# google/lyra

Measured on AMD Instinct MI355X. Metric: 20ms 16kHz frames/sec encode+decode (whole node) at batch 4096; xRT/stream, higher is better.
Workload: dtype f32+i8 (fp32 and int8 layers exactly as the reference graphs)

## Files before the change

lyra_amd/csrc/dec_kernels.hip:

```cpp
#include "dec_stages.h"

#ifdef LYRA_TIMING
extern "C" int lyra_hip_debug_exit_at_d0(int i) {
  return (int)hipMemcpyToSymbol(HIP_SYMBOL(g_lyra_exit_at), &i, sizeof(int));
}
extern "C" int lyra_hip_debug_timing_d0(long long* out) {
  return (int)hipMemcpyFromSymbol(out, HIP_SYMBOL(g_lyra_tdbg), sizeof(long long) * 128);
}
extern "C" int lyra_hip_debug_wgtrace_d0(long long* out) {
  return (int)hipMemcpyFromSymbol(out, HIP_SYMBOL(g_lyra_wgtrace), sizeof(long long) * 2048 * 4);
}
#endif

namespace lyra {

size_t dec_s0_lds_bytes() { return dec_s0_lds(); }
int dec_s0_streams_per_wg() { return SD0; }

__global__ __launch_bounds__(NTD0, I8_WAVES) void dec_s0_kernel(const DecS0P* __restrict__ Pp, const float* __restrict__ feats,
                                                       const int32_t* __restrict__ ids, int B,
                                                       uint8_t* __restrict__ state, float* __restrict__ out0,
                                                       const uint8_t* __restrict__ packets, int num_stages,
                                                       const float* __restrict__ cb, int code_bytes, int tile0) {
  LYRA_STRESS(4);
  if (((int)blockIdx.x + tile0) * SD0 >= B) return;
  dec_s0_body<0>(Pp, feats, ids, B, state, out0, packets, num_stages, cb, code_bytes, (int)blockIdx.x + tile0);
}
__global__ __launch_bounds__(NTD0, I8_WAVES) void dec_s0_dr_kernel(const DecS0P* __restrict__ Pp, const float* __restrict__ feats,
                                                          const int32_t* __restrict__ ids, int B,
                                                          uint8_t* __restrict__ state, float* __restrict__ out0,
                                                          const uint8_t* __restrict__ packets, int num_stages,
                                                          const float* __restrict__ cb, int code_bytes, int tile0) {
  LYRA_STRESS(4);
  if (((int)blockIdx.x + tile0) * SD0 >= B) return;
  dec_s0_body<1>(Pp, feats, ids, B, state, out0, packets, num_stages, cb, code_bytes, (int)blockIdx.x + tile0);
}
__global__ __launch_bounds__(NTD0, I8_WAVES) void dec_s0_bm_kernel(const DecS0P* __restrict__ Pp, const float* __restrict__ feats,
                                                          const int32_t* __restrict__ ids, int B,
                                                          uint8_t* __restrict__ state, float* __restrict__ out0,
                                                          const uint8_t* __restrict__ packets, int num_stages,
                                                          const float* __restrict__ cb, int code_bytes, int tile0) {
  LYRA_STRESS(4);
  if (((int)blockIdx.x + tile0) * SD0 >= B) return;
  dec_s0_body<3>(Pp, feats, ids, B, state, out0, packets, num_stages, cb, code_bytes, (int)blockIdx.x + tile0);
}
__global__ __launch_bounds__(NTD0, I8_WAVES) void dec_s0_xn_kernel(const DecS0P* __restrict__ Pp, const float* __restrict__ feats,
                                                          const int32_t* __restrict__ ids, int B,
                                                          uint8_t* __restrict__ state, float* __restrict__ out0,
                                                          const uint8_t* __restrict__ packets, int num_stages,
                                                          const float* __restrict__ cb, int code_bytes, int tile0) {
  LYRA_STRESS(4);
  if (((int)blockIdx.x + tile0) * SD0 >= B) return;
  dec_s0_body<2>(Pp, feats, ids, B, state, out0, packets, num_stages, cb, code_bytes, (int)blockIdx.x + tile0);
}

size_t dec_s1_lds_bytes() { return dec_s1_lds(); }
int dec_s1_streams_per_wg() { return SD1; }
int dec_s1_threads() { return NTD1; }

__global__ __launch_bounds__(NTD1, NTD1 == 512 ? 4 : 3) void dec_s1_kernel(const DecS1P* __restrict__ Pp, const float* __restrict__ in0,
                                                                          const int32_t* __restrict__ ids, int B,
                                                                          uint8_t* __restrict__ state, float* __restrict__ out1,
                                                                          int code_bytes, int tile0) {
  LYRA_STRESS(5);
  if (((int)blockIdx.x + tile0) * SD1 >= B) return;
  dec_s1_body(*Pp, in0, ids, B, state, out1, code_bytes, (int)blockIdx.x + tile0);
}

namespace {
constexpr int SD2 = S0_STREAMS;
}

size_t dec_s2_lds_bytes() { return dec_s2_lds(SD2); }
int dec_s2_streams_per_wg() { return SD2; }
int dec_s2_threads() { return 64 * SD2; }

__global__ __launch_bounds__(64 * SD2, C64_WAVES) void dec_s2_kernel(const DecS2P* __restrict__ Pp, const float* __restrict__ in1,
                                                            const int32_t* __restrict__ ids, int B,
                                                            uint8_t* __restrict__ state, int16_t* __restrict__ pcm,
                                                            int code_bytes, int tile0) {
  LYRA_STRESS(6);
  if (((int)blockIdx.x + tile0) * SD2 >= B) return;
  dec_s2_body<SD2>(*Pp, in1, ids, B, state, pcm, code_bytes, (int)blockIdx.x + tile0);
}


}
```

lyra_amd/csrc/dec_stages.h:

```cpp
#ifndef LYRA_AMD_CSRC_DEC_STAGES_H_
#define LYRA_AMD_CSRC_DEC_STAGES_H_
#include "resblock_q.h"

namespace lyra {

namespace {
constexpr int SD0 = 8;
constexpr int FS = 72;
constexpr int CS2 = 264;
constexpr int QS = 288;
constexpr int QS5 = 544;
constexpr int NTD0 = 512;
constexpr int MTD0 = (2 * SD0) / 16;
constexpr int FB_FLOATS = 3 * 16 * FS;
constexpr int XF_FLOATS = 2 * SD0 * CS2;
constexpr int H8_BYTES = 16 * QS5;
constexpr int QB_BYTES = 2 * SD0 * QS;
constexpr int QA_BYTES = 2 * 16 * QS;
constexpr int NLR = 6, NADD = 2;
static_assert(SD0 == 8, "tile size the index math below supports");
}

__host__ __device__ constexpr size_t dec_s0_lds() {
  return (size_t)(FB_FLOATS + XF_FLOATS) * 4 + H8_BYTES + 3 * QB_BYTES + QA_BYTES + 2 * SD0 * 4 + NLR * 256 +
         NADD * 2048;
}

template <int MODE>
__device__ __forceinline__ void dec_s0_body(const DecS0P* __restrict__ Pp, const float* __restrict__ feats,
                                            const int32_t* __restrict__ ids, int B, uint8_t* __restrict__ state,
                                            float* __restrict__ out0, const uint8_t* __restrict__ packets, int num_stages,
                                            const float* __restrict__ cb, int code_bytes, int tile = (int)blockIdx.x) {
  const DecS0P& P = *Pp;
  extern __shared__ __attribute__((aligned(16))) float smem[];
  float* FB = smem;
  float* XF = FB + FB_FLOATS;
  int8_t* H8 = reinterpret_cast<int8_t*>(XF + XF_FLOATS);
  int8_t* QX = H8 + H8_BYTES;
  int8_t* QA = QX + QB_BYTES;
  int8_t* QD = QA + QA_BYTES;
  int8_t* QP = QD + QB_BYTES;
  int* sids = reinterpret_cast<int*>(QP + QB_BYTES);
  int* sphase = sids + SD0;
  int32_t* LA = sphase + SD0;
  int8_t* LQ = reinterpret_cast<int8_t*>(LA + NADD * 512);
  const int tid = threadIdx.x, lane = tid & 63, wave = tid >> 6;
  const int m = lane & 15, q = lane >> 4;
  const int b0 = tile * SD0;
  LYRA_TSTAMP(80);
  LYRA_WSTAMP(120);
  LYRA_WG_BEGIN();
  if (tid < SD0) {
    int id = ids[min(b0 + tid, B - 1)];
    sids[tid] = id;
    sphase[tid] = *reinterpret_cast<const int*>(state + (size_t)max(id, 0) * st::D0_BYTES + st::PHASE);
  }
  int pkv = 0;
  const int swave = __builtin_amdgcn_readfirstlane(tid >> 6);
  if (!feats) {
    const int nbytes = (num_stages + 1) >> 1;
    const uint8_t* pk = packets + (size_t)min(b0 + swave, B - 1) * nbytes;
    if (lane < nbytes) pkv = (int)pk[lane];
  }
  load_luts<NTD0>(LQ, P.lr_lut, NLR, LA, P.add_lut, NADD);
  const auto warm = l2_warm<NTD0, 1>(P.warm);
  const auto warm_code = code_warm<NTD0>(code_bytes);
  const auto warm_cb = l2_warm<NTD0, 1>(feats ? WarmRange{nullptr, 0} : WarmRange{reinterpret_cast<const uint8_t*>(cb), 46 * 16 * 64 * 4});
  LYRA_SYNC_KEEP();
  TileCtx cx{state, sids, sphase, B - b0, st::D0_BYTES};
  const uint32_t touch0 = state_touch<SD0, NTD0>(cx, st::D_UP0, 4 * 2 * 64 * 4 + 2 * 256);
  const uint32_t touch1 = state_touch<SD0, NTD0>(cx, st::D_UP1, 2 * 2 * 64 * 4);

  {
    const int c = tid & 63, s = tid >> 6;
    const int b = min(b0 + s, B - 1);
    float f;
    if (feats) {
      f = *goff<const float>(feats + (size_t)b0 * 64, (uint32_t)(((b - b0) * 64 + c) * 4));
    } else {
      f = 0.f;
      const __amdgpu_buffer_rsrc_t cbr = __builtin_amdgcn_make_buffer_rsrc(const_cast<float*>(cb), 0, 46 * 16 * 64 * 4, 0x00020000);
#pragma unroll
      for (int k = 0; k < 46; ++k) {
        const int byte = __builtin_amdgcn_readlane(pkv, k >> 1);
        const int used = (k - num_stages) >> 31;
        const int i = (byte >> ((k & 1) ? 0 : 4)) & 15 & used;
        const float mask = __builtin_bit_cast(float, used & 0x3f800000);
        const float v = __builtin_bit_cast(float, __builtin_amdgcn_raw_buffer_load_b32(cbr, c * 4, (k * 16 + i) * 256, 0));
        f = k == 0 ? v * mask : __builtin_fmaf(v, mask, f);
      }
    }
    FB[(2 * 16 + s) * FS + at16(c)] = f;
  }
  for (int idx = tid; idx < 2 * SD0 * 16; idx += NTD0) {
    int p4 = idx & 15, s = (idx >> 4) & (SD0 - 1), j = (idx >> 4) / SD0;
    int slot = (sphase[s] + j) & 1;
    *reinterpret_cast<f32x4*>(&FB[(j * 16 + s) * FS + p4 * 4]) =
        *cx.at<const f32x4>(cx.soff(s) + (uint32_t)(st::D_HEAD + (slot * 64 + p4 * 4) * 4));
  }
  __syncthreads();
  for (int idx = tid; idx < SD0 * 16; idx += NTD0) {
    int p4 = idx & 15, s = idx >> 4;
    int slot = sphase[s] & 1;
    if (cx.valid(s))
      *cx.at<f32x4>(cx.soff(s) + (uint32_t)(st::D_HEAD + (slot * 64 + p4 * 4) * 4)) =
          *reinterpret_cast<const f32x4*>(&FB[(2 * 16 + s) * FS + p4 * 4]);
  }
  LYRA_TSTAMP(81);
  {
    f32x4 acc[1][4];
    const int g = wave >> 1;
    auto aoff = [&](int i, int c) { return (c * 16 + m) * FS + g * 16 + q * 4; };
    gemm_f32_bias<1, 4, 3, 3>(FB, aoff, P.head.w + (wave * 4) * 3 * 64, P.head.b, wave * 4 * 16, acc);
    fold_rows8<2>(acc[0]);
#pragma unroll
    for (int j = 0; j < 2; ++j) {
      int n = (wave * 4 + j + 2 * (lane >> 5)) * 16 + (lane & 15);
#pragma unroll
      for (int e = 0; e < 4; ++e)
        H8[((q & 1) * 4 + e) * QS5 + n] = (int8_t)quantize_code<MODE>(lrelu(acc[0][j][e]), P.q0);
    }
  }
  __syncthreads();
  LYRA_TSTAMP(82);
  {
    i32x4 acc[1][8];
    const int g = wave >> 1;
    const TconvQ U = P.up0[g];
    auto aoff = [&](int i, int c) { return m * QS5 + g * 128 + c * 64 + q * 16; };
    const int ct = (wave & 1) * 2 + (lane >> 5);
    const int co = ct * 16 + (lane & 15);
    const int bias = as_global(U.bias)[co];
    const float sub = as_global(P.up0_sub[g])[co];
    const int pc = at16(g * 64 + co);
    int zfv[4];
#pragma unroll
    for (int tap = 0; tap < 4; ++tap) zfv[tap] = as_global(U.zfold)[tap * 64 + co];
    float told[2][4];
#pragma unroll
    for (int e = 0; e < 4; ++e) {
      const uint32_t stp = cx.soff((q & 1) * 4 + e) + (uint32_t)(st::D_UP0 + g * 512 + co * 4);
      told[0][e] = *cx.at<const float>(stp);
      told[1][e] = *cx.at<const float>(stp + 256);
    }
    gemm_i8<1, 8, 2>(H8, aoff, U.w + ((wave & 1) * 8) * 2 * 64, acc);
    fold_rows8<4>(acc[0]);
#pragma unroll
    for (int tap = 0; tap < 4; ++tap) {
      const int zf = zfv[tap];
#pragma unroll
      for (int e = 0; e < 4; ++e) {
        const int s = (q & 1) * 4 + e;
        const uint32_t stp = cx.soff(s) + (uint32_t)(st::D_UP0 + g * 512 + co * 4);
        float y = conv_dequant<conv_flavour<MODE, false>()>(acc[0][tap][e] + zf + bias, U.M, U.sh, U.zout, P.up0_dq[g].s);
        if (tap < 2) {
          y = y + told[tap < 2 ? tap : 0][e];
          XF[(tap * SD0 + s) * CS2 + pc] = y;
        } else {
          y = y + 0.f;
          if (cx.valid(s)) *cx.at<float>(stp + (uint32_t)((tap - 2) * 256)) = y - sub;
        }
      }
    }
  }
  __syncthreads();
  LYRA_TSTAMP(83);
  const RbqPre pre1 = resblock_q_prefetch<SD0>(cx, 3, st::D_R0_1, P.dwq[1], P.pwq[1], P.cvq[1]);
  {
    const DwQ dq = P.dwq[0];
    const int w4 = tid & 63, s = tid >> 6;
    const uint32_t hp = cx.soff(s) + (uint32_t)(st::D_R0_0 + w4 * 4);
    const int h0 = *cx.at<const int>(hp), h1 = *cx.at<const int>(hp + 256);
    int ww[3];
#pragma unroll
    for (int j = 0; j < 3; ++j) ww[j] = *reinterpret_cast<const int LYRA_GLOBAL*>(&as_global(dq.w)[j * 256 + w4 * 4]);
    const i32x4 db = *reinterpret_cast<const i32x4 LYRA_GLOBAL*>(&as_global(dq.b)[w4 * 4]);
    const i32x4 dM = *reinterpret_cast<const i32x4 LYRA_GLOBAL*>(&as_global(dq.M)[w4 * 4]);
    const i32x4 dsh = *reinterpret_cast<const i32x4 LYRA_GLOBAL*>(&as_global(dq.sh)[w4 * 4]);
    int a[2];
#pragma unroll
    for (int t = 0; t < 2; ++t) {
      int c8[4];
#pragma unroll
      for (int e = 0; e < 4; ++e)
        c8[e] = quantize_code<MODE>(lrelu(XF[(t * SD0 + s) * CS2 + at16(w4 * 4 + e)]), P.q1);
      a[t] = pack8(c8[0], c8[1], c8[2], c8[3]);
    }
    const int x[2][3] = {{h0, h1, a[0]}, {h1, a[0], a[1]}};
#pragma unroll
    for (int t = 0; t < 2; ++t) {
      int o[4];
#pragma unroll
      for (int e = 0; e < 4; ++e) {
        int acc = db[e];
#pragma unroll
        for (int j = 0; j < 3; ++j) acc += sx8(x[t][j], e) * sx8(ww[j], e);
        o[e] = conv_code<conv_flavour<MODE, false>()>(acc, dM[e], dsh[e], dq.zout);
      }
      *reinterpret_cast<int*>(&QD[(t * SD0 + s) * QS + w4 * 4]) = pack8(o[0], o[1], o[2], o[3]);
      if (cx.valid(s)) *cx.at<int>(hp + (uint32_t)(t * 256)) = a[t];
    }
    __syncthreads();
    LYRA_TSTAMP(84);
    static_assert(MTD0 == 1, "one 16-row M tile: rows (t, s)");
    const int row = lane & 15, ch0 = wave * 32 + q * 4;
    {
      i32x4 acc[2] = {chan_quad(P.pwq[0].b, wave * 2), chan_quad(P.pwq[0].b, wave * 2 + 1)};
      const i32x4 M[2] = {chan_quad(P.pwq[0].M, wave * 2), chan_quad(P.pwq[0].M, wave * 2 + 1)};
      const i32x4 sh[2] = {chan_quad(P.pwq[0].sh, wave * 2), chan_quad(P.pwq[0].sh, wave * 2 + 1)};
      auto aoff = [&](int c) { return m * QS + c * 64 + q * 16; };
      gemm_i8_t<2, 4>(QD, aoff, P.pwq[0].w + (wave * 2) * 4 * 64, acc);
#pragma unroll
      for (int j = 0; j < 2; ++j) {
        int r8[4];
#pragma unroll
        for (int e = 0; e < 4; ++e) r8[e] = lut8(LQ, conv_code<conv_flavour<MODE, true>()>(acc[j][e], M[j][e], sh[j][e], P.pwq[0].zout));
        *reinterpret_cast<int*>(&QP[row * QS + ch0 + 16 * j]) = pack8(r8[0], r8[1], r8[2], r8[3]);
      }
    }
    __syncthreads();
    {
      i32x4 acc[2] = {chan_quad(P.cvq[0].b, wave * 2), chan_quad(P.cvq[0].b, wave * 2 + 1)};
      const i32x4 M[2] = {chan_quad(P.cvq[0].M, wave * 2), chan_quad(P.cvq[0].M, wave * 2 + 1)};
      const i32x4 sh[2] = {chan_quad(P.cvq[0].sh, wave * 2), chan_quad(P.cvq[0].sh, wave * 2 + 1)};
      const int g = wave >> 1;
      auto aoff = [&](int c) { return m * QS + g * 64 + q * 16; };
      gemm_i8_t<2, 1>(QP, aoff, P.cvq[0].w + (wave * 2) * 64, acc);
#pragma unroll
      for (int j = 0; j < 2; ++j) {
        int o[4];
#pragma unroll
        for (int e = 0; e < 4; ++e) {
          const float v = conv_dequant<conv_flavour<MODE, false>()>(acc[j][e], M[j][e], sh[j][e], P.cvq[0].zout, P.dq_r0.s) +
                          XF[row * CS2 + at16(ch0 + 16 * j + e)];
          o[e] = quantize_code<MODE>(v, P.q3);
        }
        *reinterpret_cast<int*>(&QX[row * QS + ch0 + 16 * j]) = pack8(o[0], o[1], o[2], o[3]);
      }
    }
    __syncthreads();
  }
  LYRA_TSTAMP(85);
  const RbqPre pre2 = resblock_q_prefetch<SD0>(cx, 9, st::D_R0_2, P.dwq[2], P.pwq[2], P.cvq[2]);
  resblock_q256<SD0, MODE>(QX, QD, QP, cx, 3, st::D_R0_1, LQ + 1 * 256, LQ + 2 * 256, P.dwq[1], P.pwq[1], P.cvq[1],
                           P.add[0], LA, pre1, 90);
  resblock_q256<SD0, MODE>(QX, QD, QP, cx, 9, st::D_R0_2, LQ + 3 * 256, LQ + 4 * 256, P.dwq[2], P.pwq[2], P.cvq[2],
                           P.add[1], LA + 512, pre2, 94);
  LYRA_TSTAMP(86);
  for (int idx = tid; idx < 2 * SD0 * 64; idx += NTD0) {
    int w4 = idx & 63, s = (idx >> 6) & (SD0 - 1), t = (idx >> 6) / SD0;
    int w = *reinterpret_cast<const int*>(&QX[(t * SD0 + s) * QS + w4 * 4]);
    *reinterpret_cast<int*>(&QA[(t * 16 + s) * QS + w4 * 4]) =
        lut8w(LQ + 5 * 256, w);
  }
  __syncthreads();
  LYRA_TSTAMP(87);
  {
    i32x4 acc[2][4];
    const int g = wave >> 2, ct = wave & 3;
    const TconvQ U = P.up1[g];
    auto aoff = [&](int i, int c) { return (i * 16 + m) * QS + g * 128 + c * 64 + q * 16; };
    gemm_i8<2, 4, 2>(QA, aoff, U.w + (ct * 4) * 2 * 64, acc);
    const int co = ct * 16 + (lane & 15);
    const int bias = as_global(U.bias)[co];
    const float sub = as_global(P.up1_sub[g])[co];
    const int pc = at16(g * 64 + co);
    int zf[4];
#pragma unroll
    for (int tap = 0; tap < 4; ++tap) zf[tap] = as_global(U.zfold)[tap * 64 + co];
#pragma unroll
    for (int e = 0; e < 4; ++e) {
      int s = q * 4 + e;
      if (s >= SD0) continue;
      const uint32_t stp = cx.soff(s) + (uint32_t)(st::D_UP1 + g * 512 + co * 4);
      int o[6];
      o[0] = acc[0][0][e] + zf[0];
      o[1] = acc[0][1][e] + zf[1];
      o[2] = (acc[0][2][e] + zf[2]) + (acc[1][0][e] + zf[0]);
      o[3] = (acc[0][3][e] + zf[3]) + (acc[1][1][e] + zf[1]);
      o[4] = acc[1][2][e] + zf[2];
      o[5] = acc[1][3][e] + zf[3];
      float y[6];
#pragma unroll
      for (int tau = 0; tau < 6; ++tau) {
        y[tau] = conv_dequant<conv_flavour<MODE, false>()>(o[tau] + bias, U.M, U.sh, U.zout, P.up1_dq[g].s);
      }
      y[0] = y[0] + *cx.at<const float>(stp);
      y[1] = y[1] + *cx.at<const float>(stp + 256);
#pragma unroll
      for (int tau = 2; tau < 6; ++tau) y[tau] = y[tau] + 0.f;
      if (cx.valid(s)) {
#pragma unroll
        for (int tau = 0; tau < 4; ++tau) *goff<float>(out0 + (size_t)b0 * 512, (uint32_t)(((s * 4 + tau) * 128 + pc) * 4)) = y[tau];
        *cx.at<float>(stp) = y[4] - sub;
        *cx.at<float>(stp + 256) = y[5] - sub;
      }
    }
  }
  LYRA_TSTAMP(88);
  LYRA_WSTAMP(121);
  LYRA_WG_END();
  if (tid < SD0 && cx.valid(tid)) {
    int ph = sphase[tid] + 1;
    *cx.at<int>(cx.soff(tid) + (uint32_t)(st::PHASE)) = ph >= st::PHASE_MOD ? 0 : ph;
  }
  l2_warm_sink(warm_cb, state, B);
  l2_warm_sink(warm, state, B);
  l2_warm_sink(warm_code, state, B);
  state_touch_sink(touch0 ^ touch1, state, B);
}

namespace {
constexpr int SD1 = 8;
constexpr int CS1 = 136;
constexpr int NTD1 = S1_THREADS;
}

namespace {
constexpr int PFB_T = PFB_DEC_S1 < 1 ? 1 : (PFB_DEC_S1 > 8 ? 8 : PFB_DEC_S1);
}
template <int NP>
struct TconvPre { f32x4 b[PFB_T][NP]; float bias[NP]; };
template <int NP>
__device__ __forceinline__ TconvPre<NP> dec_s1_tconv_wpre(const DecS1P& P, int tile0, int ntw) {
  const int lane = threadIdx.x & 63;
  const f32x4 LYRA_GLOBAL* wb = wave_uniform(P.up.w + tile0 * 16 * 64);
  TconvPre<NP> pre;
#pragma unroll
  for (int j = 0; j < NP; ++j)
    if (j < ntw) {
#pragma unroll
      for (int p = 0; p < PFB_T; ++p) pre.b[p][j] = wb[(j * 16 + p) * 64 + lane];
      pre.bias[j] = as_global(P.up.b)[((tile0 + j) * 16 + (lane & 15)) & 63];
    }
  return pre;
}
template <int NTW, int NP>
__device__ __forceinline__ void dec_s1_tconv(const float* XB, const float* SB, const DecS1P& P, const TileCtx& cx,
                                             int b0, float* __restrict__ out1, int tile0, float* HB, const TconvPre<NP>& pre) {
  static_assert(NP >= NTW, "the prefetched ring covers this wave's tiles");
  const int lane = threadIdx.x & 63;
  const int m = lane & 15, q = lane >> 4;
  f32x4 acc[2][NTW];
  auto aoff = [&](int i, int c) {
    int R = i * 16 + m, t = R / SD1, s = R & (SD1 - 1);
    return (t * SD1 + s) * CS1 + c * 16 + q * 4;
  };
  const f32x4* wfrag = P.up.w + tile0 * 16 * 64;
  {
    f32x4 bias4[NTW], wb[PFB_T][NTW];
#pragma unroll
    for (int j = 0; j < NTW; ++j) {
      const float v = pre.bias[j];
      bias4[j] = (f32x4){v, v, v, v};
#pragma unroll
      for (int p = 0; p < PFB_T; ++p) wb[p][j] = pre.b[p][j];
    }
    gemm_f32_core<2, NTW, 8, 16, 2, 1, false, PFB_T>(XB, aoff, wfrag, acc, bias4, wb);
  }
  f32x4 wb2[PFB_T][NTW];
  {
    const f32x4 LYRA_GLOBAL* w2 = wave_uniform(wfrag + 8 * 64);
#pragma unroll
    for (int p = 0; p < PFB_T; ++p)
#pragma unroll
      for (int j = 0; j < NTW; ++j) wb2[p][j] = w2[(j * 16 + p) * 64 + lane];
  }
  LYRA_TSTAMP(54);
  LYRA_WSTAMP(114);
  const bool lo = lane < 32;
#pragma unroll
  for (int j = 0; j < NTW; ++j) {
    const float biasb = as_global(P.up.b)[((tile0 + j) * 16 + (lane & 15)) & 63];
#pragma unroll
    for (int e = 0; e < 4; ++e) {
      float a = acc[0][j][e], bb = acc[1][j][e];
      HB[(j * 4 + e) * 64 + lane] = a;
      rot32_pair(a, bb);
      acc[0][j][e] = lo ? a : bb;
      acc[1][j][e] = lo ? bb : biasb;
    }
  }
  gemm_f32_cont_pre<2, NTW, 8, 16, 1, PFB_T>(XB, aoff, wfrag + 8 * 64, wb2, acc);
  LYRA_TSTAMP(55);
  LYRA_WSTAMP(115);
  int lane_e = threadIdx.x & 63;
  asm volatile("" : "+v"(lane_e));
  const int q_e = lane_e >> 4;
#pragma unroll
  for (int j = 0; j < NTW; ++j) {
    const int n = (tile0 + j) * 16 + (lane_e & 15);
    const int jj = n >> 6, co = n & 63;
    const float sub = as_global(P.up_sub)[co];
    const int pc = at16(co);
    const bool lo = lane_e < 32;
    const int blk = lo ? 0 : 1;
#pragma unroll
    for (int e = 0; e < 4; ++e) {
      const int s = (q_e & 1) * 4 + e;
      const float y0 = acc[0][j][e] + 0.f, y1 = acc[1][j][e] + 0.f;
      if (!cx.valid(s)) continue;
      float LYRA_GLOBAL* o = goff<float>(out1 + (size_t)b0 * 1280, (uint32_t)(((s * 20 + 5 * (1 + blk) + jj) * 64 + pc) * 4));
      o[0] = y0;
      if (lo) o[10 * 64] = y1;
      else *cx.at<float>(cx.soff(s) + (uint32_t)(st::D_UP2 + (jj * 64 + co) * 4)) = y1 - sub;
    }
    if (lo) {
#pragma unroll
      for (int e = 0; e < 4; ++e) {
        const int s = q_e * 4 + e;
        const float y = HB[(j * 4 + e) * 64 + lane_e] + SB[(jj * SD1 + s) * 72 + co];
        if (cx.valid(s)) *goff<float>(out1 + (size_t)b0 * 1280, (uint32_t)(((s * 20 + jj) * 64 + pc) * 4)) = y;
      }
    }
  }
}

__host__ __device__ constexpr size_t dec_s1_lds() { return (size_t)(4 * SD1 * CS1 + 4 * SD1 * CS1 + 4 * SD1 * CS1 + 5 * SD1 * 72) * 4 + 2 * SD1 * 4; }

__device__ __forceinline__ void dec_s1_body(const DecS1P& P, const float* __restrict__ in0,
                                            const int32_t* __restrict__ ids, int B, uint8_t* __restrict__ state,
                                            float* __restrict__ out1, int code_bytes, int tile = (int)blockIdx.x) {
  extern __shared__ __attribute__((aligned(16))) float smem[];
  float* XB = smem;
  float* DB = XB + 4 * SD1 * CS1;
  float* PB = DB + 4 * SD1 * CS1;
  float* SB = PB + 4 * SD1 * CS1;
  int* sids = reinterpret_cast<int*>(SB + 5 * SD1 * 72);
  int* sphase = sids + SD1;
  const int tid = threadIdx.x, wave = tid >> 6;
  const int b0 = tile * SD1;
  LYRA_TSTAMP(50);
  int my_id = 0;
  if (tid < SD1) my_id = ids[min(b0 + tid, B - 1)];
  constexpr int XIN = (4 * SD1 * 32) / NTD1;
  static_assert((4 * SD1 * 32) % NTD1 == 0 && (4 * SD1 * 32) / NTD1 >= 1, "the unrolled input prefetch covers the stage input only when the thread count divides it");
  f32x4 xin[XIN];
#pragma unroll
  for (int k = 0; k < XIN; ++k) {
    const int idx = tid + k * NTD1;
    int p4 = idx & 31, s = (idx >> 5) & (SD1 - 1), t = (idx >> 5) / SD1;
    int sb = min(s, B - 1 - b0);
    xin[k] = *goff<const f32x4>(in0 + (size_t)b0 * 512, (uint32_t)(((sb * 4 + t) * 128 + p4 * 4) * 4));
  }
  if (tid < SD1) {
    sids[tid] = my_id;
    sphase[tid] = *reinterpret_cast<const int*>(state + (size_t)max(my_id, 0) * st::D1_BYTES + st::PHASE);
  }
  const auto warm = l2_warm<NTD1, 2>(P.warm);
  const auto warm_code = code_warm<NTD1>(code_bytes);
#pragma unroll
  for (int k = 0; k < XIN; ++k) {
    const int idx = tid + k * NTD1;
    int p4 = idx & 31, s = (idx >> 5) & (SD1 - 1), t = (idx >> 5) / SD1;
    *reinterpret_cast<f32x4*>(&XB[(t * SD1 + s) * CS1 + p4 * 4]) = xin[k];
  }
  LYRA_SYNC_KEEP();
  TileCtx cx{state, sids, sphase, B - b0, st::D1_BYTES};
  const auto H0 = hist128_prefetch<SD1, NTD1>(cx, 1, st::D_R1_0);
  for (int idx = tid; idx < 5 * SD1 * 16; idx += NTD1) {
    int p4 = idx & 15, s = (idx >> 4) & (SD1 - 1), j = (idx >> 4) / SD1;
    *reinterpret_cast<f32x4*>(&SB[(j * SD1 + s) * 72 + p4 * 4]) =
        *cx.at<const f32x4>(cx.soff(s) + (uint32_t)(st::D_UP2 + (j * 64 + p4 * 4) * 4));
  }
  __syncthreads();
  LYRA_TSTAMP(51);
  LYRA_WSTAMP(111);
  resblocks128<SD1, NTD1>(XB, DB, PB, cx, P.dw, P.pw, P.cv, st::D_R1_0, st::D_R1_1, st::D_R1_2, H0);
  LYRA_TSTAMP(52);
  LYRA_WSTAMP(112);
  l2_warm_sink(warm, state, B);
  l2_warm_sink(warm_code, state, B);
  constexpr int HEAD_TILES = NTD1 == 256 ? 5 : 3;
  const bool head = NTD1 == 256 || wave < 4;
  const int tile0 = NTD1 == 256 ? wave * 5 : (head ? wave * 3 : 12 + (wave - 4) * 2);
  const auto up_pre = dec_s1_tconv_wpre<HEAD_TILES>(P, tile0, head ? HEAD_TILES : 2);
  for (int idx = tid; idx < 4 * SD1 * 32; idx += NTD1) {
    int p4 = idx & 31, rs = idx >> 5;
    f32x4* x = reinterpret_cast<f32x4*>(&XB[rs * CS1 + p4 * 4]);
    *x = lrelu4(*x);
  }
  __syncthreads();
  LYRA_TSTAMP(53);
  LYRA_WSTAMP(113);
  static_assert((NTD1 / 64) * HEAD_TILES * 256 <= 2 * 4 * SD1 * CS1, "head scratch fits into DB + PB");
  float* HB = DB + wave * (HEAD_TILES * 4 * 64);
  if (head) dec_s1_tconv<HEAD_TILES>(XB, SB, P, cx, b0, out1, tile0, HB, up_pre);
  else dec_s1_tconv<2>(XB, SB, P, cx, b0, out1, tile0, HB, up_pre);
  if (tid < SD1 && cx.valid(tid)) {
    int ph = sphase[tid] + 1;
    *cx.at<int>(cx.soff(tid) + (uint32_t)(st::PHASE)) = ph >= st::PHASE_MOD ? 0 : ph;
  }
}

namespace {
constexpr int CS0 = 72;
}
__host__ __device__ constexpr size_t dec_s2_lds(int sd2) { return (size_t)(27 * sd2 * CS0 + sd2 * 48) * 4 + 64; }

template <int SD2>
__device__ __forceinline__ void dec_s2_body(const DecS2P& P, const float* __restrict__ in1,
                                            const int32_t* __restrict__ ids, int B, uint8_t* __restrict__ state,
                                            int16_t* __restrict__ pcm, int code_bytes, int tile = (int)blockIdx.x) {
  constexpr int NTD2 = 64 * SD2;
  extern __shared__ __attribute__((aligned(16))) float smem[];
  float* XB = smem;
  float* SB = XB + 27 * SD2 * CS0;
  int* sids = reinterpret_cast<int*>(SB + SD2 * 48);
  const int tid = threadIdx.x, lane = tid & 63, wave = tid >> 6;
  const int m = lane & 15, q = lane >> 4;
  const int b0 = tile * SD2;
  LYRA_TSTAMP(60);
  int my_id = 0;
  if (tid < SD2) my_id = ids[min(b0 + tid, B - 1)];
  const int wn = wave & 3, wm = wave >> 2;
  [[maybe_unused]] const int ncol = wn * 16 + (lane & 15);
  f32x4 xr[5][1];
#pragma unroll
  for (int i = 0; i < 5; ++i) {
    const int R = (wm * 5 + i) * 16 + m, t = R / SD2, s = R & (SD2 - 1);
    const int sb = min(s, B - 1 - b0);
    xr[i][0] = *goff<const f32x4>(in1 + (size_t)b0 * 1280, (uint32_t)(((sb * 20 + t) * 64 + wn * 16 + q * 4) * 4));
  }
  if (tid < SD2) sids[tid] = my_id;
  const auto warm = l2_warm<NTD2, 1>(P.warm);
  const auto warm_code = code_warm<NTD2>(code_bytes);
  LYRA_SYNC_KEEP();
  TileCtx cx{state, sids, nullptr, B - b0, st::D2_BYTES};
  for (int idx = tid; idx < 7 * SD2 * 16; idx += NTD2) {
    int p4 = idx & 15, s = (idx >> 4) & (SD2 - 1), j = (idx >> 4) / SD2;
    int row = j < 3 ? j : 20 + j;
    *reinterpret_cast<f32x4*>(&XB[(row * SD2 + s) * CS0 + p4 * 4]) = (f32x4){0.f, 0.f, 0.f, 0.f};
  }
  for (int idx = tid; idx < SD2 * 48; idx += NTD2) {
    int s = idx / 48, i = idx - s * 48;
    SB[idx] = *cx.at<const float>(cx.soff(s) + (uint32_t)(st::D_UP3 + i * 4));
  }
  LYRA_TSTAMP(61);
  resblocks64r<SD2, NTD2>(xr, XB + 3 * SD2 * CS0, cx, P.dw, P.pw, P.cv, st::D_R2_0, st::D_R2_1, st::D_R2_2);
  LYRA_TSTAMP(62);
#pragma unroll
  for (int i = 0; i < 5; ++i)
{
    const f32x4 a4 = lrelu4(xr[i][0]);
    *reinterpret_cast<f32x4*>(&XB[(3 * SD2 + (wm * 5 + i) * 16 + m) * CS0 + wn * 16 + q * 4]) = a4;
  }
  constexpr int PFU = gemm_pf<2, 1>(), PFBU = PFB_DEC_S2 > PFU ? PFB_DEC_S2 : PFU;
  WPre<1, PFBU> up_pre;
  if (wave < 3 * SD2 / 4) {
    const f32x4 LYRA_GLOBAL* ub = wave_uniform(P.up.w);
#pragma unroll
    for (int p = 0; p < PFBU; ++p) up_pre.b[p][0] = ub[p * 64 + lane];
    const float bias = as_global(P.up.b)[0];
    up_pre.init[0] = (f32x4){bias, bias, bias, bias};
  }
  __syncthreads();
  LYRA_TSTAMP(63);
  if (wave < 3 * SD2 / 4) {
    f32x4 acc[2][1];
    auto aoff = [&](int i, int c) {
      int R = (2 * wave + i) * 16 + m, b = R / SD2, s = R & (SD2 - 1);
      return ((b + 3 - (c >> 2)) * SD2 + s) * CS0 + (c & 3) * 16 + q * 4;
    };
    gemm_f32_pre<2, 1, 16, 16, PFU, true, PFBU>(XB, aoff, P.up.w, up_pre, acc);
    LYRA_TSTAMP(64);
#pragma unroll
    for (int i = 0; i < 2; ++i) {
      const int R = (2 * wave + i) * 16 + m, b = R / SD2, s = R & (SD2 - 1);
      if (b > 22) continue;
      const int tau0 = 16 * b + 4 * q;
      f32x4 y = acc[i][0];
      f32x4 old = (f32x4){0.f, 0.f, 0.f, 0.f};
      if (tau0 < 48) old = *reinterpret_cast<const f32x4*>(&SB[s * 48 + tau0]);
#pragma unroll
      for (int e = 0; e < 4; ++e) y[e] = y[e] + old[e];
      if (!cx.valid(s)) continue;
      if (tau0 < 320) {
        int v[4];
#pragma unroll
        for (int e = 0; e < 4; ++e) {
          float f = y[e] * 32768.f;
          f = f < -32768.f ? -32768.f : f;
          f = f > 32767.f ? 32767.f : f;
          v[e] = (int)(int16_t)f;
        }
        typedef int i32x2 __attribute__((ext_vector_type(2)));
        const i32x2 pk = (i32x2){(v[0] & 0xffff) | (v[1] << 16), (v[2] & 0xffff) | (v[3] << 16)};
        *goff<i32x2>(pcm + (size_t)b0 * 320, (uint32_t)((s * 320 + tau0) * 2)) = pk;
      } else {
        f32x4 t;
#pragma unroll
        for (int e = 0; e < 4; ++e) t[e] = y[e] - P.up_sub;
        *cx.at<f32x4>(cx.soff(s) + (uint32_t)(st::D_UP3 + (tau0 - 320) * 4)) = t;
      }
    }
  }
  l2_warm_sink(warm, state, B);
  l2_warm_sink(warm_code, state, B);
}

}
#endif
```

lyra_amd/csrc/enc_kernels.hip:

```cpp
#include "enc_stages.h"

#ifdef LYRA_TIMING
extern "C" int lyra_hip_debug_exit_at_s0(int i) {
  return (int)hipMemcpyToSymbol(HIP_SYMBOL(g_lyra_exit_at), &i, sizeof(int));
}
extern "C" int lyra_hip_debug_wgtrace_s0(long long* out) {
  return (int)hipMemcpyFromSymbol(out, HIP_SYMBOL(g_lyra_wgtrace), sizeof(long long) * 2048 * 4);
}
extern "C" int lyra_hip_debug_timing(long long* out) {
  return (int)hipMemcpyFromSymbol(out, HIP_SYMBOL(g_lyra_tdbg), sizeof(long long) * 128);
}
#endif

namespace lyra {

namespace {
constexpr int S0 = S0_STREAMS;
}

size_t enc_s0_lds_bytes() { return enc_s0_lds(S0); }
int enc_s0_streams_per_wg() { return S0; }
int enc_s0_threads() { return 64 * S0; }
size_t enc_s1_lds_bytes() { return enc_s1_lds(); }
int enc_s1_streams_per_wg() { return S1; }
int enc_s1_threads() { return NT1; }

__global__ __launch_bounds__(64 * S0, C64_WAVES) void enc_s0_kernel(const EncS0P* __restrict__ Pp, const int16_t* __restrict__ pcm,
                                                           const int32_t* __restrict__ ids, int B,
                                                           uint8_t* __restrict__ state, float* __restrict__ out0,
                                                           int code_bytes, int tile0) {
  LYRA_STRESS(0);
  if (((int)blockIdx.x + tile0) * S0 >= B) return;
  enc_s0_body<S0>(*Pp, pcm, ids, B, state, out0, code_bytes, (int)blockIdx.x + tile0);
}

__global__ __launch_bounds__(NT1, NT1 == 512 ? 4 : 3) void enc_s1_kernel(const EncS1P* __restrict__ Pp, const float* __restrict__ in0,
                                                                        const int32_t* __restrict__ ids, int B,
                                                                        uint8_t* __restrict__ state, float* __restrict__ out1,
                                                                        int code_bytes, int tile0) {
  LYRA_STRESS(1);
  if (((int)blockIdx.x + tile0) * S1 >= B) return;
  enc_s1_body(*Pp, in0, ids, B, state, out1, code_bytes, (int)blockIdx.x + tile0);
}

}
```

lyra_amd/csrc/enc_s2_kernel.hip:

```cpp
#include "enc_s2_stage.h"

#ifdef LYRA_TIMING
extern "C" int lyra_hip_debug_exit_at_s2(int i) {
  return (int)hipMemcpyToSymbol(HIP_SYMBOL(g_lyra_exit_at), &i, sizeof(int));
}
extern "C" int lyra_hip_debug_timing_s2(long long* out) {
  return (int)hipMemcpyFromSymbol(out, HIP_SYMBOL(g_lyra_tdbg), sizeof(long long) * 128);
}
extern "C" int lyra_hip_debug_wgtrace_s2(long long* out) {
  return (int)hipMemcpyFromSymbol(out, HIP_SYMBOL(g_lyra_wgtrace), sizeof(long long) * 2048 * 4);
}
#endif

namespace lyra {

size_t enc_s2_lds_bytes() { return enc_s2_lds(); }
int enc_s2_streams_per_wg() { return S2; }

__global__ __launch_bounds__(NT2, I8_WAVES) void enc_s2_kernel(const EncS2P* __restrict__ Pp, const float* __restrict__ in1,
                                                      const int32_t* __restrict__ ids, int B,
                                                      uint8_t* __restrict__ state, float* __restrict__ feats,
                                                      float* __restrict__ codes_dbg, int code_bytes, int tile0) {
  LYRA_STRESS(2);
  if (((int)blockIdx.x + tile0) * S2 >= B) return;
  enc_s2_body<0>(Pp, in1, ids, B, state, feats, codes_dbg, code_bytes, (int)blockIdx.x + tile0);
}
__global__ __launch_bounds__(NT2, I8_WAVES) void enc_s2_dr_kernel(const EncS2P* __restrict__ Pp, const float* __restrict__ in1,
                                                         const int32_t* __restrict__ ids, int B,
                                                         uint8_t* __restrict__ state, float* __restrict__ feats,
                                                         float* __restrict__ codes_dbg, int code_bytes, int tile0) {
  LYRA_STRESS(2);
  if (((int)blockIdx.x + tile0) * S2 >= B) return;
  enc_s2_body<1>(Pp, in1, ids, B, state, feats, codes_dbg, code_bytes, (int)blockIdx.x + tile0);
}
__global__ __launch_bounds__(NT2, I8_WAVES) void enc_s2_bm_kernel(const EncS2P* __restrict__ Pp, const float* __restrict__ in1,
                                                         const int32_t* __restrict__ ids, int B,
                                                         uint8_t* __restrict__ state, float* __restrict__ feats,
                                                         float* __restrict__ codes_dbg, int code_bytes, int tile0) {
  LYRA_STRESS(2);
  if (((int)blockIdx.x + tile0) * S2 >= B) return;
  enc_s2_body<3>(Pp, in1, ids, B, state, feats, codes_dbg, code_bytes, (int)blockIdx.x + tile0);
}
__global__ __launch_bounds__(NT2, I8_WAVES) void enc_s2_xn_kernel(const EncS2P* __restrict__ Pp, const float* __restrict__ in1,
                                                         const int32_t* __restrict__ ids, int B,
                                                         uint8_t* __restrict__ state, float* __restrict__ feats,
                                                         float* __restrict__ codes_dbg, int code_bytes, int tile0) {
  LYRA_STRESS(2);
  if (((int)blockIdx.x + tile0) * S2 >= B) return;
  enc_s2_body<2>(Pp, in1, ids, B, state, feats, codes_dbg, code_bytes, (int)blockIdx.x + tile0);
}

}
```

lyra_amd/csrc/enc_s2_stage.h:

```cpp
#ifndef LYRA_AMD_CSRC_ENC_S2_STAGE_H_
#define LYRA_AMD_CSRC_ENC_S2_STAGE_H_
#include "resblock_q.h"

namespace lyra {

namespace {
constexpr int S2 = 8;
constexpr int CS2 = 264;
constexpr int QS = 288;
constexpr int QS5 = 544;
constexpr int NT2 = 512;
constexpr int MT2 = (2 * S2) / 16;
constexpr int XF_BYTES = 2 * S2 * CS2 * 4;
constexpr int QB_BYTES = 2 * S2 * QS;
constexpr int NLR = 7, NADD = 2;
static_assert(S2 == 8 || S2 == 16, "tile sizes the index math below supports");
static_assert(4 * S2 * QS + 16 * QS <= XF_BYTES && 3 * S2 * QS5 + 16 * QS5 <= XF_BYTES + 3 * QB_BYTES,
              "aliased int8 staging buffers (incl. the rows a partial M tile over-reads) must fit");
}

__host__ __device__ constexpr size_t enc_s2_lds() { return (size_t)2 * XF_BYTES + 3 * QB_BYTES + 2 * S2 * 4 + NLR * 256 + NADD * 2048; }

template <int MODE>
__device__ __forceinline__ void enc_s2_body(const EncS2P* __restrict__ Pp, const float* __restrict__ in1,
                                            const int32_t* __restrict__ ids, int B, uint8_t* __restrict__ state,
                                            float* __restrict__ feats, float* __restrict__ codes_dbg, int code_bytes, int tile = (int)blockIdx.x) {
  const EncS2P& P = *Pp;
  extern __shared__ __attribute__((aligned(16))) float smem[];
  float* DF = smem;
  float* XF = DF + 2 * S2 * CS2;
  int8_t* QX = reinterpret_cast<int8_t*>(XF + 2 * S2 * CS2);
  int8_t* QD = QX + QB_BYTES;
  int8_t* QP = QD + QB_BYTES;
  int* sids = reinterpret_cast<int*>(QP + QB_BYTES);
  int* sphase = sids + S2;
  int32_t* LA = sphase + S2;
  int8_t* LQ = reinterpret_cast<int8_t*>(LA + NADD * 512);
  int8_t* QB4 = reinterpret_cast<int8_t*>(DF);
  int8_t* QC = reinterpret_cast<int8_t*>(XF);
  const int tid = threadIdx.x, lane = tid & 63, wave = tid >> 6;
  const int m = lane & 15, q = lane >> 4;
  const int b0 = tile * S2;
  LYRA_TSTAMP(0);
  LYRA_WSTAMP(100);
  LYRA_WG_BEGIN();
  int my_id = 0;
  if (tid < S2) my_id = ids[min(b0 + tid, B - 1)];
  constexpr int XIN = (2 * S2 * 64) / NT2;
  static_assert((2 * S2 * 64) % NT2 == 0 && (2 * S2 * 64) / NT2 >= 1, "the unrolled input prefetch covers the stage input only when the thread count divides it");
  f32x4 xin[XIN];
#pragma unroll
  for (int k = 0; k < XIN; ++k) {
    const int idx = tid + k * NT2;
    int p4 = idx & 63, s = (idx >> 6) & (S2 - 1), t = (idx >> 6) / S2;
    int sb = min(s, B - 1 - b0);
    xin[k] = *goff<const f32x4>(in1 + (size_t)b0 * 512, (uint32_t)(((sb * 2 + t) * 256 + p4 * 4) * 4));
  }
  if (tid < S2) {
    sids[tid] = my_id;
    sphase[tid] = *reinterpret_cast<const int*>(state + (size_t)max(my_id, 0) * st::E2_BYTES + st::PHASE);
  }
  load_luts<NT2>(LQ, P.lr_lut, NLR, LA, P.add_lut, NADD);
#pragma unroll
  for (int k = 0; k < XIN; ++k) {
    const int idx = tid + k * NT2;
    int p4 = idx & 63, s = (idx >> 6) & (S2 - 1), t = (idx >> 6) / S2;
    *reinterpret_cast<f32x4*>(&XF[(t * S2 + s) * CS2 + p4 * 4]) = xin[k];
  }
  const auto warm = l2_warm<NT2, 1>(P.warm);
  const auto warm_code = code_warm<NT2>(code_bytes);
  LYRA_SYNC_KEEP();
  TileCtx cx{state, sids, sphase, B - b0, st::E2_BYTES};
  const RbqPre pre1 = resblock_q_prefetch<S2>(cx, 3, st::E_R2_1, P.dwq[0], P.pwq[0], P.cvq[0]);
  static_assert(S2 * ((st::E_R2_0 + 2048 - 1) / 128 + 1) <= NT2 && S2 * 13 <= NT2, "one touch per thread");
  const uint32_t touch0 = state_touch<S2, NT2>(cx, st::E_R2_0, 2 * 256 * 4);
  const uint32_t touch1 = state_touch<S2, NT2>(cx, st::E_D2, 2 * 256 + 2 * 512);

  __syncthreads();

  LYRA_TSTAMP(1);
  for (int idx = tid; idx < 2 * S2 * 64; idx += NT2) {
    int p4 = idx & 63, s = (idx >> 6) & (S2 - 1), t = (idx >> 6) / S2;
    f32x4 acc = {0.f, 0.f, 0.f, 0.f};
#pragma unroll
    for (int j = 0; j < 3; ++j) {
      int tau = t - (2 - j);
      f32x4 v;
      if (tau >= 0) v = lrelu4(*reinterpret_cast<const f32x4*>(&XF[(tau * S2 + s) * CS2 + p4 * 4]));
      else v = *cx.at<const f32x4>(cx.soff(s) + (uint32_t)(st::E_R2_0 + ((2 + tau) * 256 + p4 * 4) * 4));
      acc = fma4(v, *reinterpret_cast<const f32x4 LYRA_GLOBAL*>(&as_global(P.dw0.w)[j * 256 + p4 * 4]), acc);
    }
    *reinterpret_cast<f32x4*>(&DF[(t * S2 + s) * CS2 + p4 * 4]) = acc;
  }
  __syncthreads();
  for (int idx = tid; idx < 2 * S2 * 64; idx += NT2) {
    int p4 = idx & 63, s = (idx >> 6) & (S2 - 1), j = (idx >> 6) / S2;
    if (cx.valid(s))
      *cx.at<f32x4>(cx.soff(s) + (uint32_t)(st::E_R2_0 + (j * 256 + p4 * 4) * 4)) =
          lrelu4(*reinterpret_cast<const f32x4*>(&XF[(j * S2 + s) * CS2 + p4 * 4]));
  }
  LYRA_TSTAMP(2);
  {
    f32x4 acc[MT2][2];
    auto aoff = [&](int i, int c) { return (i * 16 + m) * CS2 + c * 16 + q * 4; };
    gemm_f32_bias<MT2, 2, 16, 16>(DF, aoff, P.pw0.w + (wave * 2) * 16 * 64, P.pw0.b, wave * 2 * 16, acc);
#pragma unroll
    for (int j = 0; j < 2; ++j) {
      int n = (wave * 2 + j) * 16 + (lane & 15);
#pragma unroll
      for (int i = 0; i < MT2; ++i)
#pragma unroll
        for (int e = 0; e < 4; ++e) {
          int q8 = quantize_code<MODE>(acc[i][j][e], P.q_r0);
          QP[(i * 16 + q * 4 + e) * QS + n] = (int8_t)lut8(LQ, q8);
        }
    }
  }
  __syncthreads();
  LYRA_TSTAMP(3);
  {
    static_assert(MT2 == 1, "one 16-row M tile: rows (t, s)");
    const int row = lane & 15, ch0 = wave * 32 + q * 4;
    i32x4 acc[2] = {chan_quad(P.r0b.b, wave * 2), chan_quad(P.r0b.b, wave * 2 + 1)};
    const i32x4 M[2] = {chan_quad(P.r0b.M, wave * 2), chan_quad(P.r0b.M, wave * 2 + 1)};
    const i32x4 sh[2] = {chan_quad(P.r0b.sh, wave * 2), chan_quad(P.r0b.sh, wave * 2 + 1)};
    const int g = wave >> 1;
    auto aoff = [&](int c) { return m * QS + g * 64 + q * 16; };
    gemm_i8_t<2, 1>(QP, aoff, P.r0b.w + (wave * 2) * 64, acc);
#pragma unroll
    for (int j = 0; j < 2; ++j) {
      int o[4];
#pragma unroll
      for (int e = 0; e < 4; ++e) {
        const float v = conv_dequant<conv_flavour<MODE, false>()>(acc[j][e], M[j][e], sh[j][e], P.r0b.zout, P.dq_r0.s) +
                        XF[row * CS2 + at16(ch0 + 16 * j + e)];
        o[e] = quantize_code<MODE>(v, P.q_x1);
      }
      *reinterpret_cast<int*>(&QX[row * QS + ch0 + 16 * j]) = pack8(o[0], o[1], o[2], o[3]);
    }
  }
  __syncthreads();

  LYRA_TSTAMP(4);
  const RbqPre pre2 = resblock_q_prefetch<S2>(cx, 9, st::E_R2_2, P.dwq[1], P.pwq[1], P.cvq[1]);
  resblock_q256<S2, MODE>(QX, QD, QP, cx, 3, st::E_R2_1, LQ + 1 * 256, LQ + 2 * 256, P.dwq[0], P.pwq[0], P.cvq[0],
                          P.add[0], LA, pre1, 20);
  LYRA_TSTAMP(5);
  resblock_q256<S2, MODE>(QX, QD, QP, cx, 9, st::E_R2_2, LQ + 3 * 256, LQ + 4 * 256, P.dwq[1], P.pwq[1], P.cvq[1],
                          P.add[1], LA + 512, pre2, 30);

  LYRA_TSTAMP(6);
  for (int idx = tid; idx < 2 * S2 * 64; idx += NT2) {
    int w4 = idx & 63, s = (idx >> 6) & (S2 - 1), t = (idx >> 6) / S2;
    int w = *reinterpret_cast<const int*>(&QX[(t * S2 + s) * QS + w4 * 4]);
    *reinterpret_cast<int*>(&QB4[((2 + t) * S2 + s) * QS + w4 * 4]) =
        lut8w(LQ + 5 * 256, w);
    *reinterpret_cast<int*>(&QB4[(t * S2 + s) * QS + w4 * 4]) =
        *cx.at<const int>(cx.soff(s) + (uint32_t)(st::E_D2 + t * 256 + w4 * 4));
  }
  __syncthreads();
  for (int idx = tid; idx < 2 * S2 * 64; idx += NT2) {
    int w4 = idx & 63, s = (idx >> 6) & (S2 - 1), t = (idx >> 6) / S2;
    if (cx.valid(s))
      *cx.at<int>(cx.soff(s) + (uint32_t)(st::E_D2 + t * 256 + w4 * 4)) =
          *reinterpret_cast<const int*>(&QB4[((2 + t) * S2 + s) * QS + w4 * 4]);
  }
  LYRA_TSTAMP(7);
  i32x4 dacc[1][4];
  {
    const int g = wave >> 1;
    auto aoff = [&](int i, int c) { return (c * S2 + m) * QS + g * 64 + q * 16; };
    gemm_i8<1, 4, 4>(QB4, aoff, P.down2.w + (wave * 4) * 4 * 64, dacc);
  }
  __syncthreads();
  for (int idx = tid; idx < 2 * S2 * 128; idx += NT2) {
    int w4 = idx & 127, s = (idx >> 7) & (S2 - 1), j = (idx >> 7) / S2;
    int slot = (sphase[s] + j) & 1;
    *reinterpret_cast<int*>(&QC[(j * S2 + s) * QS5 + w4 * 4]) =
        *cx.at<const int>(cx.soff(s) + (uint32_t)(st::E_BOTT + slot * 512 + w4 * 4));
  }
  fold_rows8<2>(dacc[0]);
#pragma unroll
  for (int j = 0; j < 2; ++j) {
    int n = (wave * 4 + j + 2 * (lane >> 5)) * 16 + (lane & 15);
    int bias = as_global(P.down2.b)[n], M = as_global(P.down2.M)[n], sh = as_global(P.down2.sh)[n];
#pragma unroll
    for (int e = 0; e < 4; ++e) {
      int s = (q & 1) * 4 + e;
      int c8 = conv_code<conv_flavour<MODE, false>()>(dacc[0][j][e] + bias, M, sh, P.down2.zout);
      QC[(2 * S2 + s) * QS5 + n] = (int8_t)lut8(LQ + 6 * 256, c8);
    }
  }
  __syncthreads();
  for (int idx = tid; idx < S2 * 128; idx += NT2) {
    int w4 = idx & 127, s = idx >> 7;
    int slot = sphase[s] & 1;
    if (cx.valid(s))
      *cx.at<int>(cx.soff(s) + (uint32_t)(st::E_BOTT + slot * 512 + w4 * 4)) =
          *reinterpret_cast<const int*>(&QC[(2 * S2 + s) * QS5 + w4 * 4]);
  }
  LYRA_TSTAMP(8);
  if (wave < 4) {
    i32x4 acc[1][1];
    const int g = wave;
    auto aoff = [&](int i, int c) { return ((c >> 1) * S2 + m) * QS5 + g * 128 + (c & 1) * 64 + q * 16; };
    gemm_i8<1, 1, 6>(QC, aoff, P.bott.w + g * 6 * 64, acc);
    int n = g * 16 + (lane & 15);
    int bias = as_global(P.bott.b)[n], M = as_global(P.bott.M)[n], sh = as_global(P.bott.sh)[n];
#pragma unroll
    for (int e = 0; e < 4; ++e) {
      int s = q * 4 + e;
      int c8 = conv_code<conv_flavour<MODE, false>()>(acc[0][0][e] + bias, M, sh, P.bott.zout);
      if (s < S2 && cx.valid(s)) {
        *goff<float>(feats + (size_t)b0 * 64, (uint32_t)((s * 64 + n) * 4)) = dequantize_f(c8, P.out);
        if (codes_dbg) codes_dbg[(size_t)(b0 + s) * 64 + n] = (float)c8;
      }
    }
  }
  LYRA_TSTAMP(9);
  LYRA_WSTAMP(101);
  LYRA_WG_END();
  if (tid < S2 && cx.valid(tid)) {
    int ph = sphase[tid] + 1;
    *cx.at<int>(cx.soff(tid) + (uint32_t)(st::PHASE)) = ph >= st::PHASE_MOD ? 0 : ph;
  }
  l2_warm_sink(warm, state, B);
  l2_warm_sink(warm_code, state, B);
  state_touch_sink(touch0 ^ touch1, state, B);
}

}
#endif
```

lyra_amd/csrc/enc_stages.h:

```cpp
#ifndef LYRA_AMD_CSRC_ENC_STAGES_H_
#define LYRA_AMD_CSRC_ENC_STAGES_H_
#include "resblocks.h"

namespace lyra {

namespace {
constexpr int CS0 = 72;
constexpr int PBS = 376;
constexpr int S1 = 8;
constexpr int CS1 = 136;
constexpr int NT1 = S1_THREADS;
constexpr int NW1 = NT1 / 64;
}

__host__ __device__ constexpr size_t enc_s0_lds(int s0) { return (size_t)(25 * s0 * CS0) * 4 + 64; }
__host__ __device__ constexpr size_t enc_s1_lds() { return (size_t)(6 * S1 * CS1 + 4 * S1 * CS1 + 4 * S1 * CS1) * 4 + 2 * S1 * 4; }

template <int S0>
__device__ __forceinline__ void enc_s0_body(const EncS0P& P, const int16_t* __restrict__ pcm,
                                            const int32_t* __restrict__ ids, int B, uint8_t* __restrict__ state,
                                            float* __restrict__ out0, int code_bytes, int tile = (int)blockIdx.x) {
  constexpr int NT0 = 64 * S0, NW0 = NT0 / 64;
  extern __shared__ __attribute__((aligned(16))) float smem[];
  float* XB = smem;
  int* sids = reinterpret_cast<int*>(XB + 25 * S0 * CS0);
  static_assert(S0 * PBS <= 25 * S0 * CS0, "PCM staging fits");
  const int tid = threadIdx.x, lane = tid & 63, wave = tid >> 6;
  const int m = lane & 15, q = lane >> 4;
  const int b0 = tile * S0;
  LYRA_WG_BEGIN();
  LYRA_TSTAMP(0);
  LYRA_WSTAMP(100);
  if (tid < S0) sids[tid] = ids[min(b0 + tid, B - 1)];
  const auto warm = l2_warm<NT0, 1>(P.warm);
  const auto warm_code = code_warm<NT0>(code_bytes);
  LYRA_SYNC_KEEP();
  auto soff = [&](int s) -> uint32_t { return (uint32_t)max(sids[s], 0) * (uint32_t)st::E0_BYTES; };
  auto gat = [&](uint32_t o) -> uint8_t LYRA_GLOBAL* { return (uint8_t LYRA_GLOBAL*)state + o; };
  auto valid = [&](int s) -> bool { return b0 + s < B && sids[s] >= 0; };

  f32x4 halo[2];
#pragma unroll
  for (int k = 0; k < 2; ++k) {
    const int idx = tid + k * NT0;
    const int p4 = idx & 15, s = (idx >> 4) & (S0 - 1), j = (idx >> 4) / S0;
    halo[k] = (f32x4){0.f, 0.f, 0.f, 0.f};
    if (idx < 5 * S0 * 16) halo[k] = *(const f32x4 LYRA_GLOBAL*)gat(soff(s) + (uint32_t)(st::E_D0 + (j * 64 + p4 * 4) * 4));
  }

  float* PB = XB;
  for (int idx = tid; idx < S0 * 46; idx += NT0) {
    int s = idx / 46, v = idx - s * 46;
    float x[8];
    if (v < 6) {
      const f32x4 LYRA_GLOBAL* h = (const f32x4 LYRA_GLOBAL*)gat(soff(s) + (uint32_t)(st::E_FIRST + v * 32));
      f32x4 a = h[0], b = h[1];
      x[0] = a[0]; x[1] = a[1]; x[2] = a[2]; x[3] = a[3]; x[4] = b[0]; x[5] = b[1]; x[6] = b[2]; x[7] = b[3];
    } else {
      int sb = min(s, B - 1 - b0);
      i32x4 w = *goff<const i32x4>(pcm + (size_t)b0 * 320, (uint32_t)(sb * 640 + (v - 6) * 16));
#pragma unroll
      for (int e = 0; e < 4; ++e) {
        x[2 * e] = (float)(int16_t)(w[e] & 0xffff) * (1.0f / 32768.0f);
        x[2 * e + 1] = (float)(int16_t)(w[e] >> 16) * (1.0f / 32768.0f);
      }
    }
#pragma unroll
    for (int e = 0; e < 8; ++e) PB[s * PBS + at16(v * 8 + e)] = x[e];
  }
  __syncthreads();
  for (int idx = tid; idx < S0 * 48; idx += NT0) {
    int s = idx / 48, i = idx - s * 48;
    if (valid(s)) *(float LYRA_GLOBAL*)gat(soff(s) + (uint32_t)(st::E_FIRST + i * 4)) = PB[s * PBS + at16(320 + i)];
  }
  LYRA_TSTAMP(1);

  const int wn = wave & 3, wm = wave >> 2;

  f32x4 xr[5][1];
  {
    auto aoff = [&](int i, int c) {
      int R = (wm * 5 + i) * 16 + m;
      return (R & (S0 - 1)) * PBS + (R / S0 + c) * 16 + q * 4;
    };
    gemm_f32_bias<5, 1, 4, 4, gemm_pf<5, 1>(), true>(PB, aoff, P.first.w + wn * 4 * 64, P.first.b, wn * 16, xr);
  }
  __syncthreads();
#pragma unroll
  for (int k = 0; k < 2; ++k) {
    const int idx = tid + k * NT0;
    const int p4 = idx & 15, s = (idx >> 4) & (S0 - 1), j = (idx >> 4) / S0;
    if (idx < 5 * S0 * 16) *reinterpret_cast<f32x4*>(&XB[(j * S0 + s) * CS0 + p4 * 4]) = halo[k];
  }
  LYRA_TSTAMP(2);

  TileCtx cx{state, sids, nullptr, B - b0, st::E0_BYTES};
  resblocks64r<S0, NT0>(xr, XB + 5 * S0 * CS0, cx, P.dw, P.pw, P.cv, st::E_R0_0, st::E_R0_1, st::E_R0_2);
  LYRA_TSTAMP(3);

#pragma unroll
  for (int i = 0; i < 5; ++i)
{
    const f32x4 a4 = lrelu4(xr[i][0]);
    *reinterpret_cast<f32x4*>(&XB[(5 * S0 + (wm * 5 + i) * 16 + m) * CS0 + wn * 16 + q * 4]) = a4;
  }
  constexpr int MTWE = (4 * S0) / 16, NTWE = 8 / NW0, PFE = gemm_pf<MTWE, NTWE>(), PFBE = PFB_ENC_S0 > PFE ? PFB_ENC_S0 : PFE;
  const auto down_pre = gemm_f32_wprefetch<NTWE, 40, 40, PFBE, true>(P.down.w + (wave * NTWE) * 40 * 64, P.down.b, wave * NTWE * 16);
  __syncthreads();
  for (int idx = tid; idx < 5 * S0 * 16; idx += NT0) {
    int p4 = idx & 15, s = (idx >> 4) & (S0 - 1), j = (idx >> 4) / S0;
    if (valid(s))
      *(f32x4 LYRA_GLOBAL*)gat(soff(s) + (uint32_t)(st::E_D0 + (j * 64 + p4 * 4) * 4)) =
          *reinterpret_cast<const f32x4*>(&XB[((20 + j) * S0 + s) * CS0 + p4 * 4]);
  }
  LYRA_TSTAMP(4);

  {
    constexpr int MTW = MTWE, NTW = NTWE;
    f32x4 acc[MTW][NTW];
    auto aoff = [&](int i, int c) {
      int tap = c >> 2, c16 = c & 3;
      int R = i * 16 + m;
      return ((5 * (R / S0) + tap) * S0 + (R & (S0 - 1))) * CS0 + c16 * 16 + q * 4;
    };
    gemm_f32_pre<MTW, NTW, 40, 40, PFE, true, PFBE>(XB, aoff, P.down.w + (wave * NTW) * 40 * 64, down_pre, acc);
    LYRA_TSTAMP(5);
#pragma unroll
    for (int j = 0; j < NTW; ++j) {
#pragma unroll
      for (int i = 0; i < MTW; ++i) {
        const int R = i * 16 + m, tau = R / S0, s = R & (S0 - 1);
        if (valid(s))
          *goff<f32x4>(out0 + (size_t)b0 * 512, (uint32_t)(((s * 4 + tau) * 128 + (wave * NTW + j) * 16 + q * 4) * 4)) = acc[i][j];
      }
    }
  }
  LYRA_WG_END();
  LYRA_TSTAMP(6);
  LYRA_WSTAMP(101);
  l2_warm_sink(warm, state, B);
  l2_warm_sink(warm_code, state, B);
}

__device__ __forceinline__ void enc_s1_body(const EncS1P& P, const float* __restrict__ in0,
                                            const int32_t* __restrict__ ids, int B, uint8_t* __restrict__ state,
                                            float* __restrict__ out1, int code_bytes, int tile = (int)blockIdx.x) {
  extern __shared__ __attribute__((aligned(16))) float smem[];
  float* XB = smem;
  float* DB = XB + 6 * S1 * CS1;
  float* PB = DB + 4 * S1 * CS1;
  int* sids = reinterpret_cast<int*>(PB + 4 * S1 * CS1);
  int* sphase = sids + S1;
  const int tid = threadIdx.x, lane = tid & 63, wave = tid >> 6;
  const int m = lane & 15, q = lane >> 4;
  const int b0 = tile * S1;
  LYRA_TSTAMP(70);
  LYRA_WSTAMP(102);
  int my_id = 0;
  if (tid < S1) my_id = ids[min(b0 + tid, B - 1)];
  constexpr int XIN = (4 * S1 * 32) / NT1;
  static_assert((4 * S1 * 32) % NT1 == 0 && (4 * S1 * 32) / NT1 >= 1, "the unrolled input prefetch covers the stage input only when the thread count divides it");
  f32x4 xin[XIN];
#pragma unroll
  for (int k = 0; k < XIN; ++k) {
    const int idx = tid + k * NT1;
    int p4 = idx & 31, s = (idx >> 5) & (S1 - 1), t = (idx >> 5) / S1;
    int sb = min(s, B - 1 - b0);
    xin[k] = *goff<const f32x4>(in0 + (size_t)b0 * 512, (uint32_t)(((sb * 4 + t) * 128 + p4 * 4) * 4));
  }
  if (tid < S1) {
    sids[tid] = my_id;
    sphase[tid] = *reinterpret_cast<const int*>(state + (size_t)max(my_id, 0) * st::E1_BYTES + st::PHASE);
  }
  const auto warm = l2_warm<NT1, 2>(P.warm);
  const auto warm_code = code_warm<NT1>(code_bytes);
#pragma unroll
  for (int k = 0; k < XIN; ++k) {
    const int idx = tid + k * NT1;
    int p4 = idx & 31, s = (idx >> 5) & (S1 - 1), t = (idx >> 5) / S1;
    *reinterpret_cast<f32x4*>(&XB[((2 + t) * S1 + s) * CS1 + p4 * 4]) = xin[k];
  }
  LYRA_SYNC_KEEP();
  auto soff = [&](int s) -> uint32_t { return (uint32_t)max(sids[s], 0) * (uint32_t)st::E1_BYTES; };
  auto gat = [&](uint32_t o) -> uint8_t LYRA_GLOBAL* { return (uint8_t LYRA_GLOBAL*)state + o; };
  auto valid = [&](int s) -> bool { return b0 + s < B && sids[s] >= 0; };

  TileCtx cx{state, sids, sphase, B - b0, st::E1_BYTES};
  const auto H0 = hist128_prefetch<S1, NT1>(cx, 1, st::E_R1_0);
  for (int idx = tid; idx < 2 * S1 * 32; idx += NT1) {
    int p4 = idx & 31, s = (idx >> 5) & (S1 - 1), j = (idx >> 5) / S1;
    *reinterpret_cast<f32x4*>(&XB[(j * S1 + s) * CS1 + p4 * 4]) =
        *(const f32x4 LYRA_GLOBAL*)gat(soff(s) + (uint32_t)(st::E_D1 + (j * 128 + p4 * 4) * 4));
  }
  __syncthreads();

  LYRA_TSTAMP(71);
  resblocks128<S1, NT1>(XB + 2 * S1 * CS1, DB, PB, cx, P.dw, P.pw, P.cv, st::E_R1_0, st::E_R1_1, st::E_R1_2, H0);

  LYRA_TSTAMP(72);
  l2_warm_sink(warm, state, B);
  l2_warm_sink(warm_code, state, B);
  constexpr int MTWD = (2 * S1) / 16, NTWD = 16 / NW1, PFD = gemm_pf<MTWD, NTWD>(), PFBD = PFB_ENC_S1 > PFD ? PFB_ENC_S1 : PFD;
  const auto down_pre = gemm_f32_wprefetch<NTWD, 16, 16, PFBD>(P.down.w + (wave * NTWD) * 16 * 64, P.down.b, wave * NTWD * 16);
  for (int idx = tid; idx < 4 * S1 * 32; idx += NT1) {
    int p4 = idx & 31, rs = idx >> 5;
    f32x4* x = reinterpret_cast<f32x4*>(&XB[(2 * S1 + rs) * CS1 + p4 * 4]);
    *x = lrelu4(*x);
  }
  __syncthreads();
  for (int idx = tid; idx < 2 * S1 * 32; idx += NT1) {
    int p4 = idx & 31, s = (idx >> 5) & (S1 - 1), j = (idx >> 5) / S1;
    if (valid(s))
      *(f32x4 LYRA_GLOBAL*)gat(soff(s) + (uint32_t)(st::E_D1 + (j * 128 + p4 * 4) * 4)) =
          *reinterpret_cast<const f32x4*>(&XB[((4 + j) * S1 + s) * CS1 + p4 * 4]);
  }

  {
    constexpr int MTW = MTWD, NTW = NTWD;
    f32x4 acc[MTW][NTW];
    const int nt0 = wave * NTW, g = nt0 >> 3;
    LYRA_TSTAMP(74);
    auto aoff = [&](int i, int c) {
      int tap = c >> 2, c16 = c & 3;
      int R = i * 16 + m;
      return ((2 * (R / S1) + tap) * S1 + (R & (S1 - 1))) * CS1 + g * 64 + c16 * 16 + q * 4;
    };
    gemm_f32_pre<MTW, NTW, 16, 16, PFD, false, PFBD>(XB, aoff, P.down.w + nt0 * 16 * 64, down_pre, acc);
    LYRA_TSTAMP(75);
    int lane_e = threadIdx.x & 63;
    asm volatile("" : "+v"(lane_e));
    const int q_e = lane_e >> 4;
#pragma unroll
    for (int j = 0; j < NTW; ++j) {
      const int pc = at16((nt0 + j) * 16 + (lane_e & 15));
#pragma unroll
      for (int i = 0; i < MTW; ++i)
#pragma unroll
        for (int e = 0; e < 4; ++e) {
          int R = i * 16 + q_e * 4 + e, tau = R / S1, s = R & (S1 - 1);
          if (valid(s)) *goff<float>(out1 + (size_t)b0 * 512, (uint32_t)(((s * 2 + tau) * 256 + pc) * 4)) = acc[i][j][e];
        }
    }
  }
  LYRA_TSTAMP(73);
  LYRA_WSTAMP(103);
  if (tid < S1 && valid(tid)) {
    int ph = sphase[tid] + 1;
    *(int LYRA_GLOBAL*)gat(soff(tid) + (uint32_t)st::PHASE) = ph >= st::PHASE_MOD ? 0 : ph;
  }
}

}
#endif
```

lyra_amd/csrc/kernels.h:

```cpp
#pragma once
#include "lyra_dev.h"
#include "state_layout.h"

namespace lyra {

constexpr int I8_WAVES = 4;
constexpr int C64_WAVES = 4;
constexpr int S0_STREAMS = 4;
constexpr int S1_THREADS = 512;

#ifndef LYRA_PFB_ENC_S0
#define LYRA_PFB_ENC_S0 3
#endif
#ifndef LYRA_PFB_ENC_S1
#define LYRA_PFB_ENC_S1 3
#endif
#ifndef LYRA_PFB_DEC_S1
#define LYRA_PFB_DEC_S1 2
#endif
#ifndef LYRA_PFB_DEC_S2
#define LYRA_PFB_DEC_S2 4
#endif
constexpr int PFB_ENC_S0 = LYRA_PFB_ENC_S0, PFB_ENC_S1 = LYRA_PFB_ENC_S1, PFB_DEC_S1 = LYRA_PFB_DEC_S1,
              PFB_DEC_S2 = LYRA_PFB_DEC_S2;

struct EncS0P { ConvF first; DwF dw[3]; ConvF pw[3]; ConvF cv[3]; ConvF down; WarmRange warm; };
struct EncS1P { DwF dw[3]; ConvF pw[3]; ConvF cv[3]; ConvF down; WarmRange warm; };
struct EncS2P {
  DwF dw0; ConvF pw0;
  QP q_r0, dq_r0, q_x1, out;
  LreluQ lr[7];
  const int8_t* lr_lut;
  const int32_t* add_lut;
  ConvQ r0b;
  DwQ dwq[2]; ConvQ pwq[2]; ConvQ cvq[2]; AddQ add[2];
  ConvQ down2, bott;
  int mode;
  WarmRange warm;
};

__global__ void enc_s0_kernel(const EncS0P* P, const int16_t* pcm, const int32_t* ids, int B, uint8_t* state, float* out0,
                              int code_bytes, int tile0);
__global__ void enc_s1_kernel(const EncS1P* P, const float* in0, const int32_t* ids, int B, uint8_t* state, float* out1,
                              int code_bytes, int tile0);
__global__ void enc_s2_kernel(const EncS2P* P, const float* in1, const int32_t* ids, int B, uint8_t* state, float* feats,
                              float* codes_dbg, int code_bytes, int tile0);
__global__ void enc_s2_dr_kernel(const EncS2P* P, const float* in1, const int32_t* ids, int B, uint8_t* state,
                                 float* feats, float* codes_dbg, int code_bytes, int tile0);
__global__ void enc_s2_xn_kernel(const EncS2P* P, const float* in1, const int32_t* ids, int B, uint8_t* state,
                                 float* feats, float* codes_dbg, int code_bytes, int tile0);
__global__ void enc_s2_bm_kernel(const EncS2P* P, const float* in1, const int32_t* ids, int B, uint8_t* state,
                                 float* feats, float* codes_dbg, int code_bytes, int tile0);
__global__ void enc_side_kernel(const EncS0P* P0, const EncS1P* P1, const EncS2P* P2, const int16_t* pcm, const int32_t* ids,
                                int B, uint8_t* st0, uint8_t* st1, uint8_t* st2, float* e0, float* e1, float* feats,
                                float* codes_dbg, int code_bytes);
__global__ void enc_side_dr_kernel(const EncS0P* P0, const EncS1P* P1, const EncS2P* P2, const int16_t* pcm,
                                   const int32_t* ids, int B, uint8_t* st0, uint8_t* st1, uint8_t* st2, float* e0, float* e1,
                                   float* feats, float* codes_dbg, int code_bytes);
__global__ void enc_side_xn_kernel(const EncS0P* P0, const EncS1P* P1, const EncS2P* P2, const int16_t* pcm,
                                   const int32_t* ids, int B, uint8_t* st0, uint8_t* st1, uint8_t* st2, float* e0, float* e1,
                                   float* feats, float* codes_dbg, int code_bytes);
size_t enc_side_lds_bytes();
__global__ void enc_s12_xn_kernel(const EncS1P* P1, const EncS2P* P2, const float* e0, const int32_t* ids, int B, uint8_t* st1,
                                  uint8_t* st2, float* e1, float* feats, float* codes_dbg, int code_bytes);
size_t enc_s12_lds_bytes();
size_t enc_s0_lds_bytes(); int enc_s0_streams_per_wg(); int enc_s0_threads();
size_t enc_s1_lds_bytes(); int enc_s1_streams_per_wg(); int enc_s1_threads();
size_t enc_s2_lds_bytes(); int enc_s2_streams_per_wg();

struct TconvQ { const i32x4* w; const int32_t* zfold; const int32_t* bias; int32_t M, sh, zout; };
struct DecS0P {
  ConvF head;
  QP q0;
  TconvQ up0[4]; QP up0_dq[4]; const float* up0_sub[4];
  QP q1;
  DwQ dwq[3]; ConvQ pwq[3]; ConvQ cvq[3];
  LreluQ lr[6]; AddQ add[2];
  const int8_t* lr_lut;
  const int32_t* add_lut;
  QP dq_r0, q3;
  TconvQ up1[2]; QP up1_dq[2]; const float* up1_sub[2];
  int mode;
  WarmRange warm;
};
struct DecS1P { DwF dw[3]; ConvF pw[3]; ConvF cv[3]; ConvF up; const float* up_sub; WarmRange warm; };
struct DecS2P { DwF dw[3]; ConvF pw[3]; ConvF cv[3]; ConvF up; float up_sub; WarmRange warm; };

__global__ void dec_s0_kernel(const DecS0P* P, const float* feats, const int32_t* ids, int B, uint8_t* state, float* out0,
                              const uint8_t* packets, int num_stages, const float* cb, int code_bytes, int tile0);
__global__ void dec_s0_dr_kernel(const DecS0P* P, const float* feats, const int32_t* ids, int B, uint8_t* state,
                                 float* out0, const uint8_t* packets, int num_stages, const float* cb, int code_bytes, int tile0);
__global__ void dec_s0_xn_kernel(const DecS0P* P, const float* feats, const int32_t* ids, int B, uint8_t* state,
                                 float* out0, const uint8_t* packets, int num_stages, const float* cb, int code_bytes, int tile0);
__global__ void dec_s0_bm_kernel(const DecS0P* P, const float* feats, const int32_t* ids, int B, uint8_t* state,
                                 float* out0, const uint8_t* packets, int num_stages, const float* cb, int code_bytes, int tile0);
__global__ void dec_s1_kernel(const DecS1P* P, const float* in0, const int32_t* ids, int B, uint8_t* state, float* out1,
                              int code_bytes, int tile0);
__global__ void dec_s2_kernel(const DecS2P* P, const float* in1, const int32_t* ids, int B, uint8_t* state, int16_t* pcm,
                              int code_bytes, int tile0);
__global__ void dec_side_kernel(const DecS0P* P0, const DecS1P* P1, const DecS2P* P2, const float* feats, const int32_t* ids,
                                int B, uint8_t* st0, uint8_t* st1, uint8_t* st2, float* d0, float* d1, int16_t* pcm,
                                const uint8_t* packets, int num_stages, const float* cb, int code_bytes);
__global__ void dec_side_dr_kernel(const DecS0P* P0, const DecS1P* P1, const DecS2P* P2, const float* feats,
                                   const int32_t* ids, int B, uint8_t* st0, uint8_t* st1, uint8_t* st2, float* d0, float* d1,
                                   int16_t* pcm, const uint8_t* packets, int num_stages, const float* cb, int code_bytes);
__global__ void dec_side_xn_kernel(const DecS0P* P0, const DecS1P* P1, const DecS2P* P2, const float* feats,
                                   const int32_t* ids, int B, uint8_t* st0, uint8_t* st1, uint8_t* st2, float* d0, float* d1,
                                   int16_t* pcm, const uint8_t* packets, int num_stages, const float* cb, int code_bytes);
size_t dec_side_lds_bytes();
__global__ void dec_s01_xn_kernel(const DecS0P* P0, const DecS1P* P1, const float* feats, const int32_t* ids, int B, uint8_t* st0,
                                  uint8_t* st1, float* d0, float* d1, const uint8_t* packets, int num_stages, const float* cb,
                                  int code_bytes);
size_t dec_s01_lds_bytes();
size_t dec_s0_lds_bytes(); int dec_s0_streams_per_wg();
size_t dec_s1_lds_bytes(); int dec_s1_streams_per_wg(); int dec_s1_threads();
size_t dec_s2_lds_bytes(); int dec_s2_streams_per_wg(); int dec_s2_threads();

__global__ void rvq_encode_kernel(const float* cb, const float* cbn, const float* feats, int B, int num_stages, int32_t* indices,
                                  uint8_t* packets, const int32_t* mask_ids, int32_t* packet_bytes, unsigned* stats);
__global__ void rvq_encode_chain_kernel(const float* cb, const float* feats, int B, int num_stages, int32_t* indices,
                                  uint8_t* packets, const int32_t* mask_ids, int32_t* packet_bytes);
__global__ void rvq_encode_wide_kernel(const float* cb, const float* feats, int B, int num_stages, int32_t* indices,
                                  uint8_t* packets, const int32_t* mask_ids, int32_t* packet_bytes);
__global__ void rvq_decode_kernel(const float* cb, const int32_t* indices, const uint8_t* packets, int num_stages,
                                  int B, float* feats);
__global__ void rvq_encode_mixed_kernel(const float* cb, const float* cbn, const float* feats, int B, const int32_t* bits,
                                        uint8_t* packets, const int32_t* mask_ids, int32_t* packet_bytes, unsigned* stats,
                                        unsigned* err);
__global__ void rvq_decode_mixed_kernel(const float* cb, const uint8_t* packets, const int32_t* pkt_bytes, int bytes_from_bits,
                                        int B, float* feats);
struct MelP { const double* hann; const double* tw_re; const double* tw_im; const int* band; const double* w;
              const double* wsum;
              const double* tw4_re; const double* tw4_im;
              int start, end; };
struct NoiseP { int hops_per_update; float max_smoothing, bound_decay; };
__device__ __forceinline__ float expf_via_double(float x) {
  return (float)exp((double)x);
}
__global__ void logmel_kernel(const MelP* P, const int16_t* pcm, const int32_t* ids, int B, uint8_t* state, int stride,
                              int prev_off, float* mel, int noise_tail, NoiseP NP, int32_t* is_noise_out,
                              int32_t* masked_ids);
__global__ void logmel_masked_kernel(const MelP* P, const int16_t* pcm, const int32_t* ids, int B, uint8_t* state, int stride,
                                     int prev_off, float* mel, int noise_tail, NoiseP NP, int32_t* is_noise_out,
                                     int32_t* masked_ids);
__global__ void logmel_rates_kernel(const MelP* P4, const int16_t* pcm, const int32_t* ids, const int32_t* rates, int B,
                                    uint8_t* state, int stride, int prev_off, const NoiseP* np_tab, int32_t* is_noise_out,
                                    int32_t* masked_ids);
size_t logmel_rates_lds_bytes();
__global__ void logmel_streams_kernel(const MelP* P4, const int16_t* pcm, const int32_t* ids, const int32_t* rates,
                                      const int32_t* dtx, int B, uint8_t* state, int stride, int prev_off, const NoiseP* np_tab,
                                      int32_t* is_noise_out, int32_t* masked_ids);
__global__ void noise_update_kernel(NoiseP P, const int32_t* ids, int B, uint8_t* state, const float* mel,
                                    int32_t* is_noise_out, int32_t* masked_ids);
struct ResampleP { int up, down; float coef[3][40]; };
int resample_streams_per_wg();
size_t resample_lds_bytes(int n_in);
__global__ void resample_kernel(ResampleP P, const int32_t* ids, int B, uint8_t* state, const int16_t* in, int n_in,
                                int in_stride, int16_t* out, int n_out, int out_stride);
__global__ void resample_rates_kernel(const ResampleP* tab, int dir, const int32_t* rates, const int32_t* ids, int B,
                                      uint8_t* state, const int16_t* in, int in_stride, int16_t* out, int out_stride,
                                      int32_t* ids_out, unsigned* err);
size_t resample_rates_lds_bytes();
__global__ void resample_streams_kernel(const ResampleP* tab, const int32_t* rates, const int32_t* ids, int B, uint8_t* state,
                                        const int16_t* in, const int32_t* offsets, int in_stride, long n_in_total, int16_t* out,
                                        int out_stride, int32_t* ids_out, unsigned* err);
__global__ void resample_streams_out_kernel(const ResampleP* tab, const int32_t* rates, const int32_t* ids, int B, uint8_t* state,
                                            const int16_t* in, int in_stride, int16_t* out, const int32_t* offsets,
                                            int out_stride, long n_out_total, unsigned* err);
struct TwinSlice { int32_t id, gan_off, gen_n, cng_off, cng_n, fade, fade_dir, out_off, noise_row; };
constexpr int TWIN_FADE_LO = -640, TWIN_FADE_N = 1921;
__global__ void twin_scatter_kernel(const int16_t* src, const int32_t* ids, int B, int16_t* dst);
__global__ void twin_assemble_kernel(const TwinSlice* slices, int B, const int16_t* gan, const int16_t* cng,
                                     const float* fade_w, int16_t* out, int out_stride, int16_t* noise_dense);
__device__ __forceinline__ unsigned long long splitmix64_dev(unsigned long long x) {
  x += 0x9E3779B97F4A7C15ull;
  x = (x ^ (x >> 30)) * 0xBF58476D1CE4E5B9ull;
  x = (x ^ (x >> 27)) * 0x94D049BB133111EBull;
  return x ^ (x >> 31);
}
__global__ void cng_kernel(const MelP* P, unsigned long long seed, const int32_t* ids, int B, uint8_t* state,
                           const uint8_t* noise_state, const float* features, int16_t* pcm);
__global__ void noise_read_kernel(const int32_t* ids, int B, const uint8_t* state, int field_off, float* out);
__global__ void lossy_plan_kernel(const int32_t* ids, int B, const int32_t* pkt_bytes, int nbytes, const uint8_t* rx_ring_row,
                                  uint8_t* cng_state, int32_t* gen_ids, int32_t* cng_ids, int32_t* est_ids, int32_t* info,
                                  float* feats, unsigned* err);
__global__ void lossy_plan_mixed_kernel(const int32_t* ids, int B, const int32_t* pkt_bytes, int bytes_from_bits,
                                        const uint8_t* rx_ring_row, uint8_t* cng_state, int32_t* gen_ids, int32_t* cng_ids,
                                        int32_t* est_ids, int32_t* info, float* feats, unsigned* err);
__global__ void lossy_mix_kernel(const int32_t* ids, int B, const int32_t* info, const int16_t* gan, const int16_t* cng,
                                 const float* fade_w, int16_t* out, const uint8_t* noise_state, int32_t* is_noise,
                                 int32_t* is_cn);
__global__ void bridge_mix_kernel(const int16_t* pcm, int B, const int32_t* order, const int32_t* room_start, int n_rooms,
                                  int n_members, const int32_t* muted, const int32_t* is_cn, int16_t* mix, unsigned* err);
__global__ void speakers_level_kernel(const int16_t* pcm, int B, long long* levels, int16_t* mix, int32_t* is_speaker,
                                      int32_t* pos_room, int n_members, int32_t* slot_of, int32_t* row_room);
__global__ void speakers_select_kernel(const long long* levels, int B, const int32_t* order, const int32_t* room_start,
                                       int n_rooms, int n_members, const int32_t* muted, const int32_t* is_cn,
                                       int max_speakers, unsigned long long* keys, int32_t* spk, int32_t* pos_room,
                                       int32_t* is_speaker, unsigned* err);
__global__ void speakers_mix_kernel(const int16_t* pcm, int B, const int32_t* order, int n_members, const int32_t* pos_room,
                                    int n_rooms, const int32_t* spk, int16_t* mix);
__global__ void shared_slots_kernel(const int32_t* spk, const int32_t* stream_ids, int B, const int32_t* order,
                                    const int32_t* room_start, int n_rooms, int n_members, int max_speakers,
                                    const int32_t* room_keys, int n_table_rooms, int32_t* slots, int32_t* slot_row,
                                    int32_t* slot_of, int32_t* row_room, unsigned* err);
__global__ void shared_mix_kernel(const int16_t* pcm, int B, int n_rooms, int max_speakers, const int32_t* spk,
                                  const int32_t* slot_row, const int32_t* room_keys, int n_table_rooms, int16_t* enc_mix);
__global__ void shared_fanout_kernel(int B, int n_rooms, int max_speakers, const int32_t* row_room, const int32_t* slot_of,
                                     const uint8_t* enc_packets, const int32_t* enc_packet_bytes, uint8_t* out_packets,
                                     int32_t* out_packet_bytes);
__global__ void ds_plan_kernel(const int32_t* ids, int B, const int32_t* pkt_bytes, int n_internal, uint8_t* cng_state,
                               int32_t* gen_ids, int32_t* cng1_ids, int32_t* cng2_ids, int32_t* est_ids, int32_t* info,
                               float* feats, float* ring, unsigned* err);
__global__ void ds_est_gather_kernel(const int32_t* ids, int B, const int32_t* info, const int16_t* gan_new,
                                     const int16_t* gan_held, int16_t* est_in);
__global__ void ds_slice_kernel(const int32_t* ids, int B, const int32_t* info, const int16_t* gan_new, const int16_t* cng_new,
                                int16_t* gan_held, int16_t* cng_held, const float* fade_w, int16_t* out, int out_stride,
                                const uint8_t* noise_state, int32_t* is_noise, int32_t* is_cn);
__global__ void ds_plan_any_kernel(const int32_t* ids, int B, const int32_t* pkt_bytes, int round, int n_ext, int rate,
                                   uint8_t* rs_state, int32_t* call, uint8_t* cng_state, int32_t* gen_ids, int32_t* cng1_ids,
                                   int32_t* cng2_ids, int32_t* est_ids, int32_t* info, float* feats, float* ring, unsigned* err);
size_t ds_splice_lds_bytes();
__global__ void ds_splice_kernel(ResampleP P, const int32_t* ids, int B, const int32_t* call, uint8_t* state, const int16_t* in,
                                 int in_stride, int16_t* out, int n_ext);
__global__ void ds_plan_streams_kernel(const int32_t* ids, int B, const int32_t* pkt_bytes, int round, const int32_t* rates,
                                       const int32_t* num_samples, const int32_t* offsets, int max_hops, long n_pcm_samples,
                                       uint8_t* rs_state, int32_t* call, uint8_t* cng_state, int32_t* gen_ids, int32_t* cng1_ids,
                                       int32_t* cng2_ids, int32_t* est_ids, int32_t* info, float* feats, float* ring,
                                       unsigned* err, unsigned* rates_err);
size_t ds_splice_streams_lds_bytes();
__global__ void ds_splice_streams_kernel(const ResampleP* tab, const int32_t* ids, int B, const int32_t* call, uint8_t* state,
                                         const int16_t* in, int in_stride, int16_t* out, const int32_t* offsets);
size_t logmel_lds_bytes();
size_t cng_lds_bytes();
struct ResetP { int8_t e_r2_1, e_r2_2, e_d2, e_bott, d_r0_0, d_r0_1, d_r0_2; };
__device__ __forceinline__ int reset_fill(const ResetP& P, int r, int o) {
  if (r == st::R_E2) {
    if (o >= st::E_R2_1 && o < st::E_R2_2) return P.e_r2_1;
    if (o >= st::E_R2_2 && o < st::E_D2) return P.e_r2_2;
    if (o >= st::E_D2 && o < st::E_BOTT) return P.e_d2;
    if (o >= st::E_BOTT && o < st::E_BOTT + 2 * 512) return P.e_bott;
  } else if (r == st::R_D0) {
    if (o >= st::D_R0_0 && o < st::D_R0_1) return P.d_r0_0;
    if (o >= st::D_R0_1 && o < st::D_R0_2) return P.d_r0_1;
    if (o >= st::D_R0_2 && o < st::D_UP1) return P.d_r0_2;
  }
  return 0;
}
struct StateMap { uint8_t* base[st::R_COUNT]; int bytes[st::R_COUNT]; };
__global__ void reset_kernel(const ResetP* P, const int32_t* ids, int n, int all, StateMap sm);
__global__ void state_export_kernel(const int32_t* ids, int B, int max_streams, StateMap sm, const float* ring,
                                    const int16_t* gan, const int16_t* cng, unsigned mode, unsigned long long seed,
                                    uint8_t* blobs);
__global__ void state_import_kernel(const int32_t* ids, int B, int max_streams, StateMap sm, float* ring, int16_t* gan,
                                    int16_t* cng, unsigned mode, unsigned long long seed, unsigned sides, const uint8_t* blobs,
                                    unsigned* err);
struct SpanRow { int32_t id, n_steps, n_warm, target, phase_add, handover; long long frame0; };
__global__ void span_gather_kernel(const SpanRow* rows, int B, int step, const uint8_t* frames, int row_bytes, int unit16,
                                   uint8_t* dense, int32_t* step_ids, const long long* map);
__global__ void span_scatter_kernel(const SpanRow* rows, int B, int step, const uint8_t* dense, int row_bytes, int unit16,
                                    uint8_t* frames, const long long* map);
__global__ void span_lane_init_kernel(const ResetP* P, const SpanRow* rows, int n, int r0, StateMap sm);
__global__ void span_handover_kernel(const SpanRow* rows, int n, int r0, StateMap sm);
struct SpanRsRow { long long frame0, n_frames; int32_t id, wg0, pad[2]; };
static_assert(sizeof(SpanRsRow) == sizeof(SpanRow), "one upload holds both kinds of row");
__global__ void span_resample_kernel(ResampleP P, const SpanRsRow* rows, int n_rows, uint8_t* state, const int16_t* in, int n_in,
                                     int16_t* out, int n_out);
struct SpanDtxRow { long long frame0, n_frames; int32_t id, wg0; long long region; };
static_assert(sizeof(SpanDtxRow) == sizeof(SpanRow), "one upload holds both kinds of row");
constexpr int SPAN_MEL_ROW = 164;
__global__ void span_logmel_kernel(const MelP* P, const SpanDtxRow* rows, int n_rows, uint8_t* state, const int16_t* pcm,
                                   float* mel);
__global__ void span_noise_scan_kernel(NoiseP P, const SpanDtxRow* rows, int n_rows, uint8_t* state, const float* mel,
                                       int32_t* flag_out, int v_noise, int v_active, long long* map, int32_t* counts);

struct SpanLossyRow {
  long long frame0, n_frames, info0;
  int32_t id, rx0, n_rx, rx_wg0, cng0, n_cng, cng_wg0, snap_v0;
  uint32_t ctl_out;
  int32_t pad;
};
static_assert(sizeof(SpanLossyRow) == 2 * sizeof(SpanRow), "two row slots of the upload");
struct SpanLossyRx { long long frame; int32_t snap, pad; };
struct SpanLossyCng { long long frame; int32_t snap, info; };
struct SpanLossyFrame { int32_t info, back; };
__global__ void span_lossy_ctl_read_kernel(int32_t* io, int n, int max_streams, const uint8_t* cng_state);
__global__ void span_lossy_feat_kernel(const SpanRow* rows, int B, int step, const uint8_t* gen_received, float* feats);
__global__ void span_logmel_map_kernel(const MelP* P, const SpanLossyRow* rows, int n_rows, uint8_t* state, const SpanLossyRx* rx,
                                       const int16_t* pcm, float* mel);
__global__ void span_lossy_scan_kernel(NoiseP P, const SpanLossyRow* rows, int n_rows, uint8_t* state, const float* mel,
                                       const SpanLossyRx* rx, int32_t* is_noise_out, float* snaps, int32_t* entry_noise);
__global__ void span_cng_kernel(const MelP* P, unsigned long long seed, const SpanLossyRow* rows, int n_rows, int final,
                                uint8_t* state, const SpanLossyCng* ticks, const float* snaps, const float* fade_w, int16_t* pcm16);
__global__ void span_lossy_finish_kernel(const SpanLossyRow* rows, int n_rows, long long total, const SpanLossyFrame* frames,
                                         uint8_t* cng_state, const int32_t* entry_noise, int32_t* is_noise, int32_t* is_cn);

__global__ void span_gather_mixed_kernel(const SpanRow* rows, int B, int step, const uint8_t* frames, const int32_t* frame_bits,
                                         const uint8_t* tick_bytes, uint8_t* dense, int32_t* step_ids, int32_t* step_size,
                                         const long long* map);
__global__ void span_scatter_mixed_kernel(const SpanRow* rows, int B, int step, const uint8_t* dense, const int32_t* step_bits,
                                          uint8_t* frames, int32_t* packet_bytes, const long long* map);

__global__ void span_resample_rates_kernel(const ResampleP* tab, int dir, const SpanRsRow* rows, int n_rows, uint8_t* state,
                                           const int16_t* in, int in_stride, int16_t* out, int out_stride);
__global__ void span_logmel_rates_kernel(const MelP* P4, const SpanDtxRow* rows, const SpanRsRow* rate_rows, int n_rows,
                                         uint8_t* state, const int16_t* pcm, float* mel);
__global__ void span_noise_scan_rates_kernel(const NoiseP* np_tab, const SpanDtxRow* rows, const SpanRsRow* rate_rows, int n_rows,
                                             uint8_t* state, const float* mel, int32_t* flag_out, int v_noise, int v_active,
                                             long long* map, int32_t* counts);

__global__ void span_resample_packed_kernel(const ResampleP* tab, int dir, const SpanRsRow* rows, int n_rows, uint8_t* state,
                                            const int16_t* in, int16_t* out);

}
```

lyra_amd/csrc/lyra_dev.h:

```cpp
#pragma once
#include <hip/hip_runtime.h>
#include <stdint.h>

#define LYRA_SYNC_KEEP() do { __builtin_amdgcn_fence(__ATOMIC_RELEASE, "workgroup"); __builtin_amdgcn_s_barrier(); \
                              __builtin_amdgcn_fence(__ATOMIC_ACQUIRE, "workgroup"); } while (0)

typedef float f32x4 __attribute__((ext_vector_type(4)));
typedef int i32x4 __attribute__((ext_vector_type(4)));

#define LYRA_LRELU_ALPHA 0.30000001192092896f

#ifdef LYRA_TIMING
static __device__ long long g_lyra_tdbg[128];
static __device__ int g_lyra_exit_at = -1;
#define LYRA_TSTAMP(i) do { if (blockIdx.x == 0 && threadIdx.x == 0) g_lyra_tdbg[i] = clock64(); \
    if (g_lyra_exit_at == (i)) return; } while (0)
#define LYRA_WSTAMP(i) do { if (blockIdx.x == 0 && threadIdx.x == 0) g_lyra_tdbg[i] = wall_clock64(); } while (0)
#define LYRA_TSTAMP2(i) do { if (blockIdx.x == 0 && threadIdx.x == 0) g_lyra_tdbg[i] = clock64(); } while (0)
static __device__ long long g_lyra_wgtrace[2048 * 4];
#define LYRA_WG_BEGIN() do { if (threadIdx.x == 0 && blockIdx.x < 2048) { \
    g_lyra_wgtrace[blockIdx.x * 4 + 0] = wall_clock64(); \
    g_lyra_wgtrace[blockIdx.x * 4 + 2] = __builtin_amdgcn_s_getreg(63492); \
    g_lyra_wgtrace[blockIdx.x * 4 + 3] = __builtin_amdgcn_s_getreg(63508); } } while (0)
#define LYRA_WG_END() do { if (threadIdx.x == 0 && blockIdx.x < 2048) g_lyra_wgtrace[blockIdx.x * 4 + 1] = wall_clock64(); } while (0)
#else
#define LYRA_WG_BEGIN() do { } while (0)
#define LYRA_WG_END() do { } while (0)
#define LYRA_WSTAMP(i) do { } while (0)
#define LYRA_TSTAMP(i) do { } while (0)
#define LYRA_TSTAMP2(i) do { } while (0)
#endif

#ifdef LYRA_STRESS_DELAY
#define LYRA_STRESS(bit) do { if (((LYRA_STRESS_DELAY) >> (bit)) & 1) for (int i_ = 0; i_ < 60; ++i_) __builtin_amdgcn_s_sleep(127); } while (0)
#else
#define LYRA_STRESS(bit) do { } while (0)
#endif

namespace lyra {

__host__ __device__ constexpr int at16(int k) { return (k & ~15) | ((k & 3) << 2) | ((k >> 2) & 3); }

__device__ __forceinline__ float lrelu(float x) {
  const float ax = x * LYRA_LRELU_ALPHA;
  float r;
  asm("v_max_f32 %0, %1, %2" : "=v"(r) : "v"(x), "v"(ax));
  return r;
}
typedef float f32x2 __attribute__((ext_vector_type(2)));
__device__ __forceinline__ f32x4 lrelu4(f32x4 v) {
  f32x4 r;
  const f32x2 al = (f32x2){LYRA_LRELU_ALPHA, LYRA_LRELU_ALPHA};
  f32x2 lo = (f32x2){v[0], v[1]}, hi = (f32x2){v[2], v[3]}, alo, ahi;
  alo = lo * al;
  ahi = hi * al;
  asm("v_max_f32 %0, %1, %2" : "=v"(r[0]) : "v"(v[0]), "v"(alo[0]));
  asm("v_max_f32 %0, %1, %2" : "=v"(r[1]) : "v"(v[1]), "v"(alo[1]));
  asm("v_max_f32 %0, %1, %2" : "=v"(r[2]) : "v"(v[2]), "v"(ahi[0]));
  asm("v_max_f32 %0, %1, %2" : "=v"(r[3]) : "v"(v[3]), "v"(ahi[1]));
  return r;
}
__device__ __forceinline__ f32x4 fma4(f32x4 a, f32x4 b, f32x4 c) {
  f32x4 r;
  r[0] = __builtin_fmaf(a[0], b[0], c[0]); r[1] = __builtin_fmaf(a[1], b[1], c[1]);
  r[2] = __builtin_fmaf(a[2], b[2], c[2]); r[3] = __builtin_fmaf(a[3], b[3], c[3]);
  return r;
}

__device__ __forceinline__ int32_t srdhm(int32_t a, int32_t b) {
  const int64_t p = (int64_t)a * (int64_t)b + (1ll << 30);
  return (int32_t)(p >> 31);
}
__device__ __forceinline__ int32_t rdivpot(int32_t x, int e) {
  const int32_t mask = (int32_t)((1u << e) - 1u);
  const int32_t rem = x & mask;
  const int32_t thr = (mask >> 1) + (x < 0 ? 1 : 0);
  return (x >> e) + (rem > thr ? 1 : 0);
}
__device__ __forceinline__ int32_t mbqm_double(int32_t x, int32_t M, int shift) {
  const int left = shift > 0 ? shift : 0;
  const int right = shift > 0 ? 0 : -shift;
  return rdivpot(srdhm((int32_t)((uint32_t)x << left), M), right);
}
__device__ __forceinline__ int32_t mbqm_exact(int32_t x, int32_t M, int shift) {
  int total = 31 - shift;
  return (int32_t)(((int64_t)x * (int64_t)M + (1ll << (total - 1))) >> total);
}
__device__ __forceinline__ int32_t requant(int32_t acc, int32_t M, int shift, int mode) {
  return mode ? mbqm_double(acc, M, shift) : mbqm_exact(acc, M, shift);
}
__device__ __forceinline__ int32_t clamp8(int32_t v) { return v < -128 ? -128 : (v > 127 ? 127 : v); }

struct QP { float s; int32_t z; float rs, lim; };
__device__ __forceinline__ int32_t quantize_f(float x, const QP& Q) {
  x = __builtin_fminf(__builtin_fmaxf(x, -Q.lim), Q.lim);
  const float q1 = x * Q.rs;
  const float rem = __builtin_fmaf(-q1, Q.s, x);
  const float q = __builtin_fmaf(rem, Q.rs, q1);
  return clamp8((int32_t)__builtin_roundf(q) + Q.z);
}
__device__ __forceinline__ float dequantize_f(int32_t q, float s, int32_t z) { return s * (float)(q - z); }
__device__ __forceinline__ float dequantize_f(int32_t q, const QP& Q) { return dequantize_f(q, Q.s, Q.z); }

struct LreluQ { int32_t zin, zout, mpos, spos, mneg, sneg; };
struct AddQ { int32_t z1, z2, zo, m1, s1, m2, s2, mo, so; };

__device__ __forceinline__ int32_t lrelu_q(int32_t x, const LreluQ& L) {
  int32_t v = x - L.zin;
  int32_t r = v >= 0 ? mbqm_double(v, L.mpos, L.spos) : mbqm_double(v, L.mneg, L.sneg);
  return clamp8(r + L.zout);
}
__device__ __forceinline__ int32_t add_q(int32_t a, int32_t b, const AddQ& L) {
  int32_t va = (a - L.z1) * (1 << 20);
  int32_t vb = (b - L.z2) * (1 << 20);
  int32_t sa = mbqm_double(va, L.m1, L.s1);
  int32_t sb = mbqm_double(vb, L.m2, L.s2);
  return clamp8(mbqm_double(sa + sb, L.mo, L.so) + L.zo);
}

__device__ __forceinline__ int32_t rne_clamped_code(float v, int32_t z) {
  const float lo = (float)(-128 - z), hi = (float)(127 - z);
  const float c = __builtin_amdgcn_fmed3f(v, lo, hi);
  return __float_as_int(c + 12582912.f) - (0x4B400000 - z);
}
__device__ __forceinline__ int32_t xnn_requant(int32_t acc, int32_t Mbits, int32_t zout) {
  return rne_clamped_code((float)acc * __int_as_float(Mbits), zout);
}
template <int MODE, bool UNGROUPED_CONV>
__host__ __device__ constexpr int conv_flavour() { return MODE == 3 ? (UNGROUPED_CONV ? 0 : 1) : MODE; }
template <int MODE>
__device__ __forceinline__ int32_t conv_code(int32_t acc, int32_t M, int sh, int32_t zout) {
  static_assert(MODE >= 0 && MODE <= 2, "a layer's flavour (conv_flavour<>), not the kernel's mode");
  if constexpr (MODE == 2) return xnn_requant(acc, M, zout);
  else return clamp8(requant(acc, M, sh, MODE) + zout);
}
template <int MODE>
__device__ __forceinline__ float conv_dequant(int32_t acc, int32_t M, int sh, int32_t zout, float s_dq) {
  if constexpr (MODE == 2) {
    const float lo = (float)(-128 - zout), hi = (float)(127 - zout);
    const float c = __builtin_amdgcn_fmed3f((float)acc * __int_as_float(M), lo, hi);
    const float r = (c + 12582912.f) - 12582912.f;
    return s_dq * r;
  } else {
    return dequantize_f(conv_code<MODE>(acc, M, sh, zout), s_dq, zout);
  }
}
__device__ __forceinline__ int32_t xnn_quantize(float x, const QP& Q) { return rne_clamped_code(x * Q.rs, Q.z); }
template <int MODE>
__device__ __forceinline__ int32_t quantize_code(float x, const QP& Q) {
  if constexpr (MODE == 2) return xnn_quantize(x, Q);
  else return quantize_f(x, Q);
}
__device__ __forceinline__ int32_t xnn_add(int32_t a, int32_t b, const AddQ& L) {
  const int32_t acc = L.mo + a * L.m1 + b * L.m2;
  return clamp8((acc >> L.so) + L.zo);
}

#define LYRA_GLOBAL __attribute__((address_space(1)))
template <class T>
__device__ __forceinline__ const T LYRA_GLOBAL* as_global(const T* p) {
  return (const T LYRA_GLOBAL*)p;
}
template <class T, class U>
__device__ __forceinline__ T LYRA_GLOBAL* goff(U* base, uint32_t byte_off) {
  return (T LYRA_GLOBAL*)((uint8_t LYRA_GLOBAL*)base + byte_off);
}
template <class T>
__device__ __forceinline__ const T LYRA_GLOBAL* wave_uniform(const T* p) {
  const uint64_t v = (uint64_t)p;
  const uint32_t lo = __builtin_amdgcn_readfirstlane((uint32_t)v), hi = __builtin_amdgcn_readfirstlane((uint32_t)(v >> 32));
  return (const T LYRA_GLOBAL*)(((uint64_t)hi << 32) | lo);
}

template <int NTW, int PF>
struct WPre { f32x4 b[PF][NTW]; f32x4 init[NTW]; };

__device__ __forceinline__ f32x4 bias_quad(const float* bias, int n0) {
  return *reinterpret_cast<const f32x4 LYRA_GLOBAL*>(as_global(bias) + n0 + (((threadIdx.x & 63) >> 4) << 2));
}

template <int NTW, int KC, int KS, int PF, bool SWAP = false>
__device__ __forceinline__ WPre<NTW, PF> gemm_f32_wprefetch(const f32x4* bfrag_generic, const float* bias, int n0) {
  const int lane = threadIdx.x & 63;
  const f32x4 LYRA_GLOBAL* bbase = wave_uniform(bfrag_generic);
  WPre<NTW, PF> pre;
#pragma unroll
  for (int p = 0; p < PF; ++p)
#pragma unroll
    for (int j = 0; j < NTW; ++j) pre.b[p][j] = bbase[(j * KS + (p < KC ? p : 0)) * 64 + lane];
  if constexpr (SWAP) {
#pragma unroll
    for (int j = 0; j < NTW; ++j) pre.init[j] = bias_quad(bias, n0 + j * 16);
  } else {
    const float LYRA_GLOBAL* b = as_global(bias) + n0 + (threadIdx.x & 15);
#pragma unroll
    for (int j = 0; j < NTW; ++j) {
      const float v = b[j * 16];
      pre.init[j] = (f32x4){v, v, v, v};
    }
  }
  return pre;
}

template <int MTW, int NTW, int KC, int KS, int INIT, int PF, bool SWAP = false, int PFB = PF, class AOff>
__device__ __forceinline__ void gemm_f32_core(const float* lds, AOff a_off, const f32x4* bfrag_generic,
                                              f32x4 (&acc)[MTW][NTW], const f32x4 (&init)[NTW],
                                              const f32x4 (*pre_b)[NTW] = nullptr) {
  static_assert(PFB >= PF && PF >= 1, "the weight ring is at least as deep as the activation ring");
  const int lane = threadIdx.x & 63;
  const f32x4 LYRA_GLOBAL* bbase = wave_uniform(bfrag_generic);
  if (INIT == 2) {
#pragma unroll
    for (int j = 0; j < NTW; ++j) acc[MTW - 1][j] = init[j];
  }
  f32x4 bq[PFB + 1][NTW], aq[PF + 1][MTW];
#pragma unroll
  for (int p = 0; p < PFB; ++p)
    if (p < KC) {
#pragma unroll
      for (int j = 0; j < NTW; ++j) bq[p][j] = pre_b ? pre_b[p][j] : bbase[(j * KS + p) * 64 + lane];
      if (p < PF) {
#pragma unroll
        for (int i = 0; i < MTW; ++i) aq[p][i] = *reinterpret_cast<const f32x4*>(lds + a_off(i, p));
      }
    }
#pragma unroll
  for (int c = 0; c < KC; ++c) {
    if (c + PFB < KC) {
      const int sl = (c + PFB) % (PFB + 1);
#pragma unroll
      for (int j = 0; j < NTW; ++j) bq[sl][j] = bbase[(j * KS + (c + PFB)) * 64 + lane];
    }
    if (c + PF < KC) {
      const int sl = (c + PF) % (PF + 1);
#pragma unroll
      for (int i = 0; i < MTW; ++i) aq[sl][i] = *reinterpret_cast<const f32x4*>(lds + a_off(i, c + PF));
    }
    if constexpr (PFB > PF) __builtin_amdgcn_sched_barrier(0);
    const int cb = c % (PFB + 1), ca = c % (PF + 1);
#pragma unroll
    for (int kk = 0; kk < 4; ++kk)
#pragma unroll
      for (int i = 0; i < MTW; ++i)
#pragma unroll
        for (int j = 0; j < NTW; ++j) {
          const bool first = c == 0 && kk == 0;
          const f32x4 cin = (first && INIT == 0) ? (f32x4){0.f, 0.f, 0.f, 0.f} : (first && INIT == 2) ? acc[MTW - 1][j] : acc[i][j];
          acc[i][j] = SWAP ? __builtin_amdgcn_mfma_f32_16x16x4f32(bq[cb][j][kk], aq[ca][i][kk], cin, 0, 0, 0)
                           : __builtin_amdgcn_mfma_f32_16x16x4f32(aq[ca][i][kk], bq[cb][j][kk], cin, 0, 0, 0);
        }
  }
}

template <int MTW, int NTW, int KC, int KS = KC, bool ZERO = true,
          int PF = (4 * MTW * NTW >= 16 ? 1 : (4 * MTW * NTW >= 8 ? 2 : 3)), class AOff>
__device__ __forceinline__ void gemm_f32(const float* lds, AOff a_off, const f32x4* bfrag_generic,
                                         f32x4 (&acc)[MTW][NTW]) {
  f32x4 none[NTW];
  gemm_f32_core<MTW, NTW, KC, KS, ZERO ? 0 : 1, PF>(lds, a_off, bfrag_generic, acc, none);
}
template <int MTW, int NTW, int KC, int KS, int PF, int PFB, class AOff>
__device__ __forceinline__ void gemm_f32_cont_pre(const float* lds, AOff a_off, const f32x4* bfrag_generic,
                                                  const f32x4 (&pre_b)[PFB][NTW], f32x4 (&acc)[MTW][NTW]) {
  f32x4 none[NTW];
  gemm_f32_core<MTW, NTW, KC, KS, 1, PF, false, PFB>(lds, a_off, bfrag_generic, acc, none, pre_b);
}

template <int MTW, int NTW, int KC, int KS = KC,
          int PF = (4 * MTW * NTW >= 16 ? 1 : (4 * MTW * NTW >= 8 ? 2 : 3)), bool SWAP = false, class AOff>
__device__ __forceinline__ void gemm_f32_bias(const float* lds, AOff a_off, const f32x4* bfrag_generic,
                                              const float* bias, int n0, f32x4 (&acc)[MTW][NTW]) {
  f32x4 init[NTW];
  if constexpr (SWAP) {
#pragma unroll
    for (int j = 0; j < NTW; ++j) init[j] = bias_quad(bias, n0 + j * 16);
  } else {
    const float LYRA_GLOBAL* b = as_global(bias) + n0 + (threadIdx.x & 15);
#pragma unroll
    for (int j = 0; j < NTW; ++j) {
      const float v = b[j * 16];
      init[j] = (f32x4){v, v, v, v};
    }
  }
  gemm_f32_core<MTW, NTW, KC, KS, 2, PF, SWAP>(lds, a_off, bfrag_generic, acc, init);
}

template <int MTW, int NTW, int KC, int KS = KC,
          int PF = (4 * MTW * NTW >= 16 ? 1 : (4 * MTW * NTW >= 8 ? 2 : 3)), bool SWAP = false, int PFB = PF, class AOff>
__device__ __forceinline__ void gemm_f32_pre(const float* lds, AOff a_off, const f32x4* bfrag_generic,
                                             const WPre<NTW, PFB>& pre, f32x4 (&acc)[MTW][NTW]) {
  gemm_f32_core<MTW, NTW, KC, KS, 2, PF, SWAP, PFB>(lds, a_off, bfrag_generic, acc, pre.init, pre.b);
}
template <int MTW, int NTW>
constexpr int gemm_pf() { return 4 * MTW * NTW >= 16 ? 1 : (4 * MTW * NTW >= 8 ? 2 : 3); }

template <int MTW, int NTW, int KC, int KS = KC,
          int PF = (4 * MTW * NTW >= 16 ? 1 : (4 * MTW * NTW >= 8 ? 2 : 3)), bool SWAP = false, class AOff>
__device__ __forceinline__ void gemm_f32_init(const float* lds, AOff a_off, const f32x4* bfrag_generic,
                                              const f32x4 (&init)[NTW], f32x4 (&acc)[MTW][NTW]) {
  gemm_f32_core<MTW, NTW, KC, KS, 2, PF, SWAP>(lds, a_off, bfrag_generic, acc, init);
}

template <int MTW, int NTW, int KC, class AOff>
__device__ __forceinline__ void gemm_i8(const int8_t* lds, AOff a_off, const i32x4* bfrag_generic,
                                        i32x4 (&acc)[MTW][NTW]) {
  const int lane = threadIdx.x & 63;
  const i32x4 LYRA_GLOBAL* bfrag = wave_uniform(bfrag_generic);
#pragma unroll
  for (int i = 0; i < MTW; ++i)
#pragma unroll
    for (int j = 0; j < NTW; ++j) acc[i][j] = (i32x4){0, 0, 0, 0};
#pragma unroll
  for (int c = 0; c < KC; ++c) {
    i32x4 b[NTW], a[MTW];
#pragma unroll
    for (int j = 0; j < NTW; ++j) b[j] = bfrag[(j * KC + c) * 64 + lane];
#pragma unroll
    for (int i = 0; i < MTW; ++i) a[i] = *reinterpret_cast<const i32x4*>(lds + a_off(i, c));
#pragma unroll
    for (int i = 0; i < MTW; ++i)
#pragma unroll
      for (int j = 0; j < NTW; ++j)
        acc[i][j] = __builtin_amdgcn_mfma_i32_16x16x64_i8(a[i], b[j], acc[i][j], 0, 0, 0);
  }
}

template <int NTW, int KC, class AOff>
__device__ __forceinline__ void gemm_i8_t(const int8_t* lds, AOff a_off, const i32x4* bfrag_generic, i32x4 (&acc)[NTW]) {
  const int lane = threadIdx.x & 63;
  const i32x4 LYRA_GLOBAL* bfrag = wave_uniform(bfrag_generic);
#pragma unroll
  for (int c = 0; c < KC; ++c) {
    i32x4 w[NTW];
#pragma unroll
    for (int j = 0; j < NTW; ++j) w[j] = bfrag[(j * KC + c) * 64 + lane];
    const i32x4 a = *reinterpret_cast<const i32x4*>(lds + a_off(c));
#pragma unroll
    for (int j = 0; j < NTW; ++j) acc[j] = __builtin_amdgcn_mfma_i32_16x16x64_i8(w[j], a, acc[j], 0, 0, 0);
  }
}
__device__ __forceinline__ i32x4 chan_quad(const int32_t* p, int nt) {
  return *reinterpret_cast<const i32x4 LYRA_GLOBAL*>(as_global(p) + nt * 16 + (((threadIdx.x & 63) >> 4) << 2));
}

template <int H>
__device__ __forceinline__ void fold_rows8(i32x4 (&acc)[2 * H]) {
#pragma unroll
  for (int j = 0; j < H; ++j)
#pragma unroll
    for (int e = 0; e < 4; ++e)
      acc[j][e] = (int)__builtin_amdgcn_permlane32_swap((unsigned)acc[j][e], (unsigned)acc[j + H][e], false, false)[0];
}
template <int H>
__device__ __forceinline__ void fold_rows8(f32x4 (&acc)[2 * H]) {
#pragma unroll
  for (int j = 0; j < H; ++j)
#pragma unroll
    for (int e = 0; e < 4; ++e)
      acc[j][e] = __uint_as_float(__builtin_amdgcn_permlane32_swap(__float_as_uint(acc[j][e]),
                                                                   __float_as_uint(acc[j + H][e]), false, false)[0]);
}

__device__ __forceinline__ void rot32_pair(float& a, float& b) {
  auto r1 = __builtin_amdgcn_permlane32_swap(__float_as_uint(a), __float_as_uint(b), false, false);
  auto r2 = __builtin_amdgcn_permlane32_swap(r1[1], r1[0], false, false);
  a = __uint_as_float(r2[0]);
  b = __uint_as_float(r2[1]);
}

__device__ __forceinline__ int cd_col() { return threadIdx.x & 15; }
__device__ __forceinline__ int cd_row(int reg) { return (((threadIdx.x & 63) >> 4) << 2) + reg; }

struct ConvF { const f32x4* w; const float* b; };
struct DwF { const float* w; const float* b; };
struct ConvQ { const i32x4* w; const int32_t* b; const int32_t* M; const int32_t* sh; int32_t zout; };
struct DwQ { const int8_t* w; const int32_t* b; const int32_t* M; const int32_t* sh; int32_t zin, zout; };

struct WarmRange { const uint8_t* base; uint32_t bytes; };

template <int MAXIT>
struct WarmTok { uint32_t v[MAXIT]; };

template <int NT, int MAXIT>
__device__ __forceinline__ WarmTok<MAXIT> l2_warm(const WarmRange& w) {
  const uint32_t lines = w.bytes >> 7;
  const uint32_t wgs = (gridDim.x + 7) >> 3, me = blockIdx.x >> 3;
  const uint32_t per = (lines + wgs - 1) / wgs;
  const uint32_t lo = me * per;
  uint32_t hi = lo + per;
  hi = hi < lines ? hi : lines;
  WarmTok<MAXIT> tok;
#pragma unroll
  for (int it = 0; it < MAXIT; ++it) {
    const uint32_t l = lo + it * NT + threadIdx.x;
    tok.v[it] = 0;
    if (l < hi) tok.v[it] = *reinterpret_cast<const uint32_t LYRA_GLOBAL*>(as_global(w.base) + ((size_t)l << 7));
  }
  return tok;
}
template <int NT>
__device__ __forceinline__ WarmTok<1> code_warm(int code_bytes) {
  const uint64_t pc = __builtin_amdgcn_s_getpc();
  return l2_warm<NT, 1>(WarmRange{reinterpret_cast<const uint8_t*>(pc & ~127ull), (uint32_t)(code_bytes > 0 ? code_bytes : 0)});
}

template <int MAXIT>
__device__ __forceinline__ void l2_warm_sink(const WarmTok<MAXIT>& tok, uint8_t* state, int B) {
  uint32_t acc = 0;
#pragma unroll
  for (int it = 0; it < MAXIT; ++it) acc ^= tok.v[it];
  if (acc == 0x9E3779B9u && B == -0x5EED) state[0] = (uint8_t)acc;
}

}
```

lyra_amd/csrc/resblocks.h:

```cpp
#pragma once
#include "kernels.h"

namespace lyra {

struct TileCtx {
  uint8_t* state;
  const int* sids;
  const int* sphase;
  int nvalid;
  int stride;
  __device__ __forceinline__ uint8_t* sbase(int s) const { return state + (size_t)max(sids[s], 0) * stride; }
  __device__ __forceinline__ bool valid(int s) const { return s < nvalid && sids[s] >= 0; }
  __device__ __forceinline__ uint32_t soff(int s) const { return (uint32_t)max(sids[s], 0) * (uint32_t)stride; }
  template <class T>
  __device__ __forceinline__ T LYRA_GLOBAL* at(uint32_t byte_off) const {
    return (T LYRA_GLOBAL*)((uint8_t LYRA_GLOBAL*)state + byte_off);
  }
};

template <int S, int NT>
__device__ __forceinline__ uint32_t state_touch(const TileCtx& cx, int off, int bytes) {
  const int l0 = off >> 7, n = ((off + bytes - 1) >> 7) - l0 + 1;
  const int idx = threadIdx.x;
  uint32_t tok = 0;
  if (idx < S * n) {
    const int s = idx / n, l = idx - s * n;
    tok = *cx.at<const uint32_t>(cx.soff(s) + (uint32_t)((l0 + l) << 7));
  }
  return tok;
}
__device__ __forceinline__ void state_touch_sink(uint32_t tok, uint8_t* state, int B) {
  if (tok == 0x9E3779B9u && B == -0x5EED) state[0] = (uint8_t)tok;
}

template <int S, int NT>
__device__ __forceinline__ void resblocks64r(f32x4 (&xr)[5][1], float* A, const TileCtx& cx, const DwF* dws,
                                             const ConvF* pws, const ConvF* cvs, int off0, int off1, int off2) {
  constexpr int CS = 72;
  static_assert(20 * S / 16 == 5 * (NT / 256), "5 M tiles per wave");
#pragma unroll 1
  for (int r = 0; r < 3; ++r) {
    int tid = threadIdx.x;
    asm volatile("" : "+v"(tid));
    const int lane = tid & 63, wave = tid >> 6;
    const int m = lane & 15, q = lane >> 4;
    const int wn = wave & 3, wm = wave >> 2;
    [[maybe_unused]] const int ncol = wn * 16 + (lane & 15);
    const int d = r == 0 ? 1 : (r == 1 ? 3 : 9);
    const int R2 = 2 * d;
    const int off = r == 0 ? off0 : (r == 1 ? off1 : off2);
    LYRA_TSTAMP(10 + r * 8 + 0);
    constexpr int RSTEP = NT / 16;
    const int p4 = tid & 15, rq = tid >> 4;
    const float LYRA_GLOBAL* dww = as_global(dws[r].w);
    static_assert(RSTEP % S == 0, "one stream per thread");
    constexpr int TSTEP = RSTEP / S;
    const int sq = rq & (S - 1), tq = rq / S;
    const uint32_t hb0 = cx.soff(sq) + (uint32_t)(off + (tq * 64 + p4 * 4) * 4);
    const uint32_t hb1 = hb0 + (uint32_t)(d * 256);
    f32x4 h0[5], h1[5];
#pragma unroll
    for (int k = 0; k < 5; ++k) {
      const int t = tq + k * TSTEP;
      h0[k] = (f32x4){0.f, 0.f, 0.f, 0.f};
      h1[k] = (f32x4){0.f, 0.f, 0.f, 0.f};
      if (t < 2 * d) h0[k] = *cx.at<const f32x4>(hb0 + k * TSTEP * 256);
      if (t < d) h1[k] = *cx.at<const f32x4>(hb1 + k * TSTEP * 256);
    }
#pragma unroll
    for (int i = 0; i < 5; ++i)
{
      const f32x4 a4 = lrelu4(xr[i][0]);
      *reinterpret_cast<f32x4*>(&A[((wm * 5 + i) * 16 + m) * CS + wn * 16 + q * 4]) = a4;
    }
    __syncthreads();
    LYRA_TSTAMP(10 + r * 8 + 1);
    f32x4 dreg[5];
    {
      const f32x4 w0 = *reinterpret_cast<const f32x4 LYRA_GLOBAL*>(dww + p4 * 4);
#pragma unroll
      for (int k = 0; k < 5; ++k) {
        const int t0 = tq + k * TSTEP - 2 * d;
        const f32x4 v0 = t0 >= 0 ? *reinterpret_cast<const f32x4*>(&A[(t0 * S + sq) * CS + p4 * 4]) : h0[k];
        dreg[k] = fma4(v0, w0, (f32x4){0.f, 0.f, 0.f, 0.f});
      }
      const f32x4 w1 = *reinterpret_cast<const f32x4 LYRA_GLOBAL*>(dww + 64 + p4 * 4);
#pragma unroll
      for (int k = 0; k < 5; ++k) {
        const int t1 = tq + k * TSTEP - d;
        const f32x4 v1 = t1 >= 0 ? *reinterpret_cast<const f32x4*>(&A[(t1 * S + sq) * CS + p4 * 4]) : h1[k];
        dreg[k] = fma4(v1, w1, dreg[k]);
      }
      const f32x4 w2 = *reinterpret_cast<const f32x4 LYRA_GLOBAL*>(dww + 128 + p4 * 4);
#pragma unroll
      for (int k = 0; k < 5; ++k) {
        const f32x4 v2 = *reinterpret_cast<const f32x4*>(&A[(rq + k * RSTEP) * CS + p4 * 4]);
        dreg[k] = fma4(v2, w2, dreg[k]);
      }
    }
    LYRA_TSTAMP(10 + r * 8 + 2);
    __syncthreads();
#pragma unroll
    for (int k = 0; k < 5; ++k) {
      f32x4* item = reinterpret_cast<f32x4*>(&A[(rq + k * RSTEP) * CS + p4 * 4]);
      const int j = tq + k * TSTEP - (20 - R2);
      if (j >= 0 && cx.valid(sq)) *cx.at<f32x4>(cx.soff(sq) + (uint32_t)(off + (j * 64 + p4 * 4) * 4)) = *item;
      *item = dreg[k];
    }
    __syncthreads();
    LYRA_TSTAMP(10 + r * 8 + 4);
    auto aoff = [&](int i, int c) { return ((wm * 5 + i) * 16 + m) * CS + c * 16 + q * 4; };
    WPre<1, 1> cv_pre;
    {
      f32x4 acc[5][1];
      gemm_f32_bias<5, 1, 4, 4, gemm_pf<5, 1>(), true>(A, aoff, pws[r].w + wn * 4 * 64, pws[r].b, wn * 16, acc);
      LYRA_TSTAMP(10 + r * 8 + 5);
      cv_pre = gemm_f32_wprefetch<1, 4, 4, 1, true>(cvs[r].w + wn * 4 * 64, cvs[r].b, wn * 16);
      __syncthreads();
#pragma unroll
      for (int i = 0; i < 5; ++i)
{
        const f32x4 a4 = lrelu4(acc[i][0]);
        *reinterpret_cast<f32x4*>(&A[((wm * 5 + i) * 16 + m) * CS + wn * 16 + q * 4]) = a4;
      }
      __syncthreads();
      LYRA_TSTAMP(10 + r * 8 + 6);
    }
    {
      f32x4 acc[5][1];
      gemm_f32_pre<5, 1, 4, 4, gemm_pf<5, 1>(), true>(A, aoff, cvs[r].w + wn * 4 * 64, cv_pre, acc);
#pragma unroll
      for (int i = 0; i < 5; ++i)
#pragma unroll
        for (int e = 0; e < 4; ++e) xr[i][0][e] = acc[i][0][e] + xr[i][0][e];
    }
    LYRA_TSTAMP(10 + r * 8 + 7);
    __syncthreads();
  }
}

template <int RPT>
struct Hist128 { f32x4 h[RPT][2]; };

template <int S, int NT>
__device__ __forceinline__ Hist128<1024 / NT> hist128_prefetch(const TileCtx& cx, int d, int off) {
  constexpr int RPT = 1024 / NT;
  const int tid = threadIdx.x, p4 = tid & 31, s = (tid >> 5) & (S - 1), row0 = (tid >> 8) * RPT;
  const int R2 = 2 * d;
  const bool ring = R2 > 4;
  const int base = ring ? (cx.sphase[s] * 4) % R2 : 0;
  const uint32_t hp = cx.soff(s) + (uint32_t)(off + p4 * 16);
  Hist128<RPT> H;
#pragma unroll
  for (int k = 0; k < RPT; ++k)
#pragma unroll
    for (int j = 0; j < 2; ++j) {
      const int tau = row0 + k - (2 - j) * d;
      H.h[k][j] = (f32x4){0.f, 0.f, 0.f, 0.f};
      if (tau < 0) {
        int row = R2 + tau;
        if (ring) { row = base + tau + R2; row = row >= R2 ? row - R2 : row; }
        H.h[k][j] = *cx.at<const f32x4>(hp + (uint32_t)(row * 512));
      }
    }
  return H;
}

template <int S, int NT>
__device__ __forceinline__ void resblocks128(float* X, float* D, float* P, const TileCtx& cx, const DwF* dws,
                                             const ConvF* pws, const ConvF* cvs, int off0, int off1, int off2,
                                             Hist128<1024 / NT> H) {
  static_assert(S == 8 && (NT == 256 || NT == 512), "thread <-> (stream, channel quad, row half) mapping");
  constexpr int CS = 136, NTW = 8 / (NT / 64), MT = 2, RPT = 1024 / NT;
  constexpr int PF = gemm_pf<MT, NTW>();
#pragma unroll 1
  for (int r = 0; r < 3; ++r) {
    int tid = threadIdx.x;
    asm volatile("" : "+v"(tid));
    const int lane = tid & 63, wave = tid >> 6;
    const int m = lane & 15, q = lane >> 4;
    const int p4 = tid & 31, s = (tid >> 5) & (S - 1), row0 = (tid >> 8) * RPT;
    const int d = r == 0 ? 1 : (r == 1 ? 3 : 9);
    const int R2 = 2 * d;
    const int off = r == 0 ? off0 : (r == 1 ? off1 : off2);
    const bool ring = R2 > 4;
    LYRA_TSTAMP(40 + r * 8 + 0);
    {
      const float LYRA_GLOBAL* dww = as_global(dws[r].w) + p4 * 4;
      const f32x4 w0 = *reinterpret_cast<const f32x4 LYRA_GLOBAL*>(dww);
      const f32x4 w1 = *reinterpret_cast<const f32x4 LYRA_GLOBAL*>(dww + 128);
      const f32x4 w2 = *reinterpret_cast<const f32x4 LYRA_GLOBAL*>(dww + 256);
      const uint32_t hp = cx.soff(s) + (uint32_t)(off + p4 * 16);
      const int base = ring ? (cx.sphase[s] * 4) % R2 : 0;
      const bool valid = cx.valid(s);
      const float* xq = &X[s * CS + p4 * 4];
#pragma unroll
      for (int k = 0; k < RPT; ++k) {
        const int t = row0 + k, t0 = t - 2 * d, t1 = t - d;
        const f32x4 a = lrelu4(*reinterpret_cast<const f32x4*>(xq + t * S * CS));
        f32x4 v0 = H.h[k][0], v1 = H.h[k][1];
        if (t0 >= 0) v0 = lrelu4(*reinterpret_cast<const f32x4*>(xq + t0 * S * CS));
        if (t1 >= 0) v1 = lrelu4(*reinterpret_cast<const f32x4*>(xq + t1 * S * CS));
        f32x4 acc = fma4(v0, w0, (f32x4){0.f, 0.f, 0.f, 0.f});
        acc = fma4(v1, w1, acc);
        acc = fma4(a, w2, acc);
        *reinterpret_cast<f32x4*>(&D[(t * S + s) * CS + p4 * 4]) = acc;
        if (valid) {
          if (ring) {
            int row = base + t;
            row = row >= R2 ? row - R2 : row;
            *cx.at<f32x4>(hp + (uint32_t)(row * 512)) = a;
          } else if (t >= 2) {
            *cx.at<f32x4>(hp + (uint32_t)((t - 2) * 512)) = a;
          }
        }
      }
    }
    const auto pw_pre = gemm_f32_wprefetch<NTW, 8, 8, PF>(pws[r].w + (wave * NTW) * 8 * 64, pws[r].b, wave * NTW * 16);
    WPre<NTW, PF> cv_pre;
    __syncthreads();
    LYRA_TSTAMP(40 + r * 8 + 2);
    {
      f32x4 acc[MT][NTW];
      auto aoff = [&](int i, int c) { return (i * 16 + m) * CS + c * 16 + q * 4; };
      gemm_f32_pre<MT, NTW, 8, 8, PF>(D, aoff, pws[r].w + (wave * NTW) * 8 * 64, pw_pre, acc);
      cv_pre = gemm_f32_wprefetch<NTW, 4, 4, PF>(cvs[r].w + (wave * NTW) * 4 * 64, cvs[r].b, wave * NTW * 16);
      LYRA_TSTAMP(40 + r * 8 + 3);
      if (r < 2) H = hist128_prefetch<S, NT>(cx, r == 0 ? 3 : 9, r == 0 ? off1 : off2);
#pragma unroll
      for (int j = 0; j < NTW; ++j) {
        const int ncol = (wave * NTW + j) * 16 + (lane & 15);
        const int pcol = at16(ncol);
#pragma unroll
        for (int i = 0; i < MT; ++i) {
          const f32x4 a4 = lrelu4(acc[i][j]);
#pragma unroll
          for (int e = 0; e < 4; ++e) P[(i * 16 + q * 4 + e) * CS + pcol] = a4[e];
        }
      }
      __syncthreads();
      LYRA_TSTAMP(40 + r * 8 + 4);
    }
    {
      f32x4 acc[MT][NTW];
      const int g = (wave * NTW) >> 2;
      auto aoff = [&](int i, int c) { return (i * 16 + m) * CS + g * 64 + c * 16 + q * 4; };
      gemm_f32_pre<MT, NTW, 4, 4, PF>(P, aoff, cvs[r].w + (wave * NTW) * 4 * 64, cv_pre, acc);
      LYRA_TSTAMP(40 + r * 8 + 5);
#pragma unroll
      for (int j = 0; j < NTW; ++j) {
        const int ncol = (wave * NTW + j) * 16 + (lane & 15);
        const int pcol = at16(ncol);
#pragma unroll
        for (int i = 0; i < MT; ++i)
#pragma unroll
          for (int e = 0; e < 4; ++e) {
            float* x = &X[(i * 16 + q * 4 + e) * CS + pcol];
            *x = acc[i][j][e] + *x;
          }
      }
    }
    __syncthreads();
    LYRA_TSTAMP(40 + r * 8 + 6);
  }
}

}
```

Measured before the change: 14.45 million.

## Issue per-stream state loads before the LDS barrier using slot ids read directly from global

In the enc_s1, enc_s2 and dec_s1 stage prologues, each thread now reads its stream id straight from global ids and computes its own state offset. This lets the history, delay and upsample loads go out before the shared-memory id table is published and the first barrier completes. In enc_s2 the depthwise history and weights are held in registers, the pw0 GEMM weight prefetch is issued earlier, and one redundant state touch and one barrier are removed. It also adds head-timing debug stamps, which are compiled out by default. The cost is higher register pressure and extra global id loads per thread.

```diff
diff --git a/lyra_amd/csrc/dec_kernels.hip b/lyra_amd/csrc/dec_kernels.hip
--- a/lyra_amd/csrc/dec_kernels.hip
+++ b/lyra_amd/csrc/dec_kernels.hip
@@ -9,6 +9,9 @@
 }
 extern "C" int lyra_hip_debug_wgtrace_d0(long long* out) {
   return (int)hipMemcpyFromSymbol(out, HIP_SYMBOL(g_lyra_wgtrace), sizeof(long long) * 2048 * 4);
+}
+extern "C" int lyra_hip_debug_heads_dec(long long* out) {
+  return (int)hipMemcpyFromSymbol(out, HIP_SYMBOL(g_lyra_heads), sizeof(long long) * 3 * 128 * 4);
 }
 #endif
 
diff --git a/lyra_amd/csrc/dec_stages.h b/lyra_amd/csrc/dec_stages.h
--- a/lyra_amd/csrc/dec_stages.h
+++ b/lyra_amd/csrc/dec_stages.h
@@ -48,6 +48,7 @@
   const int m = lane & 15, q = lane >> 4;
   const int b0 = tile * SD0;
   LYRA_TSTAMP(80);
+  LYRA_HSTAMP(0, 0);
   LYRA_WSTAMP(120);
   LYRA_WG_BEGIN();
   if (tid < SD0) {
@@ -107,6 +108,7 @@
           *reinterpret_cast<const f32x4*>(&FB[(2 * 16 + s) * FS + p4 * 4]);
   }
   LYRA_TSTAMP(81);
+  LYRA_HSTAMP(0, 1);
   {
     f32x4 acc[1][4];
     const int g = wave >> 1;
@@ -298,6 +300,7 @@
     }
   }
   LYRA_TSTAMP(88);
+  LYRA_HSTAMP(0, 2);
   LYRA_WSTAMP(121);
   LYRA_WG_END();
   if (tid < SD0 && cx.valid(tid)) {
@@ -431,8 +434,11 @@
   const int tid = threadIdx.x, wave = tid >> 6;
   const int b0 = tile * SD1;
   LYRA_TSTAMP(50);
+  LYRA_HSTAMP(1, 0);
   int my_id = 0;
   if (tid < SD1) my_id = ids[min(b0 + tid, B - 1)];
+  const int id_me = slot_id(ids, b0, (tid >> 5) & (SD1 - 1), B);
+  const int id_sb = slot_id(ids, b0, (tid >> 4) & (SD1 - 1), B);
   constexpr int XIN = (4 * SD1 * 32) / NTD1;
   static_assert((4 * SD1 * 32) % NTD1 == 0 && (4 * SD1 * 32) / NTD1 >= 1, "the unrolled input prefetch covers the stage input only when the thread count divides it");
   f32x4 xin[XIN];
@@ -447,6 +453,21 @@
     sids[tid] = my_id;
     sphase[tid] = *reinterpret_cast<const int*>(state + (size_t)max(my_id, 0) * st::D1_BYTES + st::PHASE);
   }
+  TileCtx cx{state, sids, sphase, B - b0, st::D1_BYTES};
+  const auto H0 = hist128_prefetch_at<SD1, NTD1>(cx, slot_off(id_me, st::D1_BYTES), 0, 1, st::D_R1_0);
+  constexpr int TIN = (5 * SD1 * 16 + NTD1 - 1) / NTD1;
+  static_assert((NTD1 >> 4) % SD1 == 0, "one slot per thread");
+  f32x4 tin[TIN];
+  {
+    const uint32_t so_sb = slot_off(id_sb, st::D1_BYTES);
+#pragma unroll
+    for (int k = 0; k < TIN; ++k) {
+      const int idx = tid + k * NTD1;
+      int p4 = idx & 15, j = (idx >> 4) / SD1;
+      tin[k] = (f32x4){0.f, 0.f, 0.f, 0.f};
+      if (idx < 5 * SD1 * 16) tin[k] = *cx.at<const f32x4>(so_sb + (uint32_t)(st::D_UP2 + (j * 64 + p4 * 4) * 4));
+    }
+  }
   const auto warm = l2_warm<NTD1, 2>(P.warm);
   const auto warm_code = code_warm<NTD1>(code_bytes);
 #pragma unroll
@@ -455,16 +476,15 @@
     int p4 = idx & 31, s = (idx >> 5) & (SD1 - 1), t = (idx >> 5) / SD1;
     *reinterpret_cast<f32x4*>(&XB[(t * SD1 + s) * CS1 + p4 * 4]) = xin[k];
   }
+#pragma unroll
+  for (int k = 0; k < TIN; ++k) {
+    const int idx = tid + k * NTD1;
+    int p4 = idx & 15, s = (idx >> 4) & (SD1 - 1), j = (idx >> 4) / SD1;
+    if (idx < 5 * SD1 * 16) *reinterpret_cast<f32x4*>(&SB[(j * SD1 + s) * 72 + p4 * 4]) = tin[k];
+  }
   LYRA_SYNC_KEEP();
-  TileCtx cx{state, sids, sphase, B - b0, st::D1_BYTES};
-  const auto H0 = hist128_prefetch<SD1, NTD1>(cx, 1, st::D_R1_0);
-  for (int idx = tid; idx < 5 * SD1 * 16; idx += NTD1) {
-    int p4 = idx & 15, s = (idx >> 4) & (SD1 - 1), j = (idx >> 4) / SD1;
-    *reinterpret_cast<f32x4*>(&SB[(j * SD1 + s) * 72 + p4 * 4]) =
-        *cx.at<const f32x4>(cx.soff(s) + (uint32_t)(st::D_UP2 + (j * 64 + p4 * 4) * 4));
-  }
-  __syncthreads();
   LYRA_TSTAMP(51);
+  LYRA_HSTAMP(1, 1);
   LYRA_WSTAMP(111);
   resblocks128<SD1, NTD1>(XB, DB, PB, cx, P.dw, P.pw, P.cv, st::D_R1_0, st::D_R1_1, st::D_R1_2, H0);
   LYRA_TSTAMP(52);
@@ -487,6 +507,7 @@
   float* HB = DB + wave * (HEAD_TILES * 4 * 64);
   if (head) dec_s1_tconv<HEAD_TILES>(XB, SB, P, cx, b0, out1, tile0, HB, up_pre);
   else dec_s1_tconv<2>(XB, SB, P, cx, b0, out1, tile0, HB, up_pre);
+  LYRA_HSTAMP(1, 2);
   if (tid < SD1 && cx.valid(tid)) {
     int ph = sphase[tid] + 1;
     *cx.at<int>(cx.soff(tid) + (uint32_t)(st::PHASE)) = ph >= st::PHASE_MOD ? 0 : ph;
@@ -511,6 +532,7 @@
   const int m = lane & 15, q = lane >> 4;
   const int b0 = tile * SD2;
   LYRA_TSTAMP(60);
+  LYRA_HSTAMP(2, 0);
   int my_id = 0;
   if (tid < SD2) my_id = ids[min(b0 + tid, B - 1)];
   const int wn = wave & 3, wm = wave >> 2;
@@ -537,6 +559,7 @@
     SB[idx] = *cx.at<const float>(cx.soff(s) + (uint32_t)(st::D_UP3 + i * 4));
   }
   LYRA_TSTAMP(61);
+  LYRA_HSTAMP(2, 1);
   resblocks64r<SD2, NTD2>(xr, XB + 3 * SD2 * CS0, cx, P.dw, P.pw, P.cv, st::D_R2_0, st::D_R2_1, st::D_R2_2);
   LYRA_TSTAMP(62);
 #pragma unroll
@@ -595,6 +618,7 @@
       }
     }
   }
+  LYRA_HSTAMP(2, 2);
   l2_warm_sink(warm, state, B);
   l2_warm_sink(warm_code, state, B);
 }
diff --git a/lyra_amd/csrc/enc_kernels.hip b/lyra_amd/csrc/enc_kernels.hip
--- a/lyra_amd/csrc/enc_kernels.hip
+++ b/lyra_amd/csrc/enc_kernels.hip
@@ -9,6 +9,9 @@
 }
 extern "C" int lyra_hip_debug_timing(long long* out) {
   return (int)hipMemcpyFromSymbol(out, HIP_SYMBOL(g_lyra_tdbg), sizeof(long long) * 128);
+}
+extern "C" int lyra_hip_debug_heads_enc(long long* out) {
+  return (int)hipMemcpyFromSymbol(out, HIP_SYMBOL(g_lyra_heads), sizeof(long long) * 3 * 128 * 4);
 }
 #endif
 
diff --git a/lyra_amd/csrc/enc_s2_kernel.hip b/lyra_amd/csrc/enc_s2_kernel.hip
--- a/lyra_amd/csrc/enc_s2_kernel.hip
+++ b/lyra_amd/csrc/enc_s2_kernel.hip
@@ -9,6 +9,9 @@
 }
 extern "C" int lyra_hip_debug_wgtrace_s2(long long* out) {
   return (int)hipMemcpyFromSymbol(out, HIP_SYMBOL(g_lyra_wgtrace), sizeof(long long) * 2048 * 4);
+}
+extern "C" int lyra_hip_debug_heads_s2(long long* out) {
+  return (int)hipMemcpyFromSymbol(out, HIP_SYMBOL(g_lyra_heads), sizeof(long long) * 3 * 128 * 4);
 }
 #endif
 
diff --git a/lyra_amd/csrc/enc_s2_stage.h b/lyra_amd/csrc/enc_s2_stage.h
--- a/lyra_amd/csrc/enc_s2_stage.h
+++ b/lyra_amd/csrc/enc_s2_stage.h
@@ -42,10 +42,12 @@
   const int m = lane & 15, q = lane >> 4;
   const int b0 = tile * S2;
   LYRA_TSTAMP(0);
+  LYRA_HSTAMP(0, 0);
   LYRA_WSTAMP(100);
   LYRA_WG_BEGIN();
   int my_id = 0;
   if (tid < S2) my_id = ids[min(b0 + tid, B - 1)];
+  const int id_me = slot_id(ids, b0, (tid >> 6) & (S2 - 1), B);
   constexpr int XIN = (2 * S2 * 64) / NT2;
   static_assert((2 * S2 * 64) % NT2 == 0 && (2 * S2 * 64) / NT2 >= 1, "the unrolled input prefetch covers the stage input only when the thread count divides it");
   f32x4 xin[XIN];
@@ -60,6 +62,19 @@
     sids[tid] = my_id;
     sphase[tid] = *reinterpret_cast<const int*>(state + (size_t)max(my_id, 0) * st::E2_BYTES + st::PHASE);
   }
+  TileCtx cx{state, sids, sphase, B - b0, st::E2_BYTES};
+  static_assert(NT2 == 64 * S2, "thread = (slot, channel quad); idx + NT2 is the next time step of the same item");
+  f32x4 hr[2];
+  {
+    const uint32_t so_me = slot_off(id_me, st::E2_BYTES);
+#pragma unroll
+    for (int j = 0; j < 2; ++j) hr[j] = *cx.at<const f32x4>(so_me + (uint32_t)(st::E_R2_0 + (j * 256 + (tid & 63) * 4) * 4));
+  }
+  f32x4 dw0w[3];
+#pragma unroll
+  for (int j = 0; j < 3; ++j) dw0w[j] = *reinterpret_cast<const f32x4 LYRA_GLOBAL*>(&as_global(P.dw0.w)[j * 256 + (tid & 63) * 4]);
+  static_assert(S2 * 13 <= NT2, "one touch per thread");
+  const uint32_t touch1 = state_touch_head<S2, NT2>(state, ids, b0, B, st::E2_BYTES, st::E_D2, 2 * 256 + 2 * 512);
   load_luts<NT2>(LQ, P.lr_lut, NLR, LA, P.add_lut, NADD);
 #pragma unroll
   for (int k = 0; k < XIN; ++k) {
@@ -70,29 +85,27 @@
   const auto warm = l2_warm<NT2, 1>(P.warm);
   const auto warm_code = code_warm<NT2>(code_bytes);
   LYRA_SYNC_KEEP();
-  TileCtx cx{state, sids, sphase, B - b0, st::E2_BYTES};
-  const RbqPre pre1 = resblock_q_prefetch<S2>(cx, 3, st::E_R2_1, P.dwq[0], P.pwq[0], P.cvq[0]);
-  static_assert(S2 * ((st::E_R2_0 + 2048 - 1) / 128 + 1) <= NT2 && S2 * 13 <= NT2, "one touch per thread");
-  const uint32_t touch0 = state_touch<S2, NT2>(cx, st::E_R2_0, 2 * 256 * 4);
-  const uint32_t touch1 = state_touch<S2, NT2>(cx, st::E_D2, 2 * 256 + 2 * 512);
-
-  __syncthreads();
 
   LYRA_TSTAMP(1);
-  for (int idx = tid; idx < 2 * S2 * 64; idx += NT2) {
-    int p4 = idx & 63, s = (idx >> 6) & (S2 - 1), t = (idx >> 6) / S2;
+#pragma unroll
+  for (int t = 0; t < 2; ++t) {
+    const int p4 = tid & 63, s = tid >> 6;
     f32x4 acc = {0.f, 0.f, 0.f, 0.f};
 #pragma unroll
     for (int j = 0; j < 3; ++j) {
-      int tau = t - (2 - j);
+      const int tau = t - (2 - j);
       f32x4 v;
       if (tau >= 0) v = lrelu4(*reinterpret_cast<const f32x4*>(&XF[(tau * S2 + s) * CS2 + p4 * 4]));
-      else v = *cx.at<const f32x4>(cx.soff(s) + (uint32_t)(st::E_R2_0 + ((2 + tau) * 256 + p4 * 4) * 4));
-      acc = fma4(v, *reinterpret_cast<const f32x4 LYRA_GLOBAL*>(&as_global(P.dw0.w)[j * 256 + p4 * 4]), acc);
+      else v = hr[2 + tau];
+      acc = fma4(v, dw0w[j], acc);
     }
     *reinterpret_cast<f32x4*>(&DF[(t * S2 + s) * CS2 + p4 * 4]) = acc;
   }
-  __syncthreads();
+  constexpr int PFP = gemm_pf<MT2, 2>(), PFBP = PFB_ENC_S2 > PFP ? PFB_ENC_S2 : PFP;
+  const auto pw0_pre = gemm_f32_wprefetch<2, 16, 16, PFBP>(P.pw0.w + (wave * 2) * 16 * 64, P.pw0.b, wave * 2 * 16);
+  const RbqPre pre1 = resblock_q_prefetch<S2>(cx, 3, st::E_R2_1, P.dwq[0], P.pwq[0], P.cvq[0]);
+  __syncthreads();
+  LYRA_HSTAMP(0, 1);
   for (int idx = tid; idx < 2 * S2 * 64; idx += NT2) {
     int p4 = idx & 63, s = (idx >> 6) & (S2 - 1), j = (idx >> 6) / S2;
     if (cx.valid(s))
@@ -103,7 +116,7 @@
   {
     f32x4 acc[MT2][2];
     auto aoff = [&](int i, int c) { return (i * 16 + m) * CS2 + c * 16 + q * 4; };
-    gemm_f32_bias<MT2, 2, 16, 16>(DF, aoff, P.pw0.w + (wave * 2) * 16 * 64, P.pw0.b, wave * 2 * 16, acc);
+    gemm_f32_pre<MT2, 2, 16, 16, PFP, false, PFBP>(DF, aoff, P.pw0.w + (wave * 2) * 16 * 64, pw0_pre, acc);
 #pragma unroll
     for (int j = 0; j < 2; ++j) {
       int n = (wave * 2 + j) * 16 + (lane & 15);
@@ -218,6 +231,7 @@
     }
   }
   LYRA_TSTAMP(9);
+  LYRA_HSTAMP(0, 2);
   LYRA_WSTAMP(101);
   LYRA_WG_END();
   if (tid < S2 && cx.valid(tid)) {
@@ -226,7 +240,7 @@
   }
   l2_warm_sink(warm, state, B);
   l2_warm_sink(warm_code, state, B);
-  state_touch_sink(touch0 ^ touch1, state, B);
+  state_touch_sink(touch1, state, B);
 }
 
 }
diff --git a/lyra_amd/csrc/enc_stages.h b/lyra_amd/csrc/enc_stages.h
--- a/lyra_amd/csrc/enc_stages.h
+++ b/lyra_amd/csrc/enc_stages.h
@@ -30,6 +30,7 @@
   const int b0 = tile * S0;
   LYRA_WG_BEGIN();
   LYRA_TSTAMP(0);
+  LYRA_HSTAMP(0, 0);
   LYRA_WSTAMP(100);
   if (tid < S0) sids[tid] = ids[min(b0 + tid, B - 1)];
   const auto warm = l2_warm<NT0, 1>(P.warm);
@@ -74,6 +75,7 @@
     if (valid(s)) *(float LYRA_GLOBAL*)gat(soff(s) + (uint32_t)(st::E_FIRST + i * 4)) = PB[s * PBS + at16(320 + i)];
   }
   LYRA_TSTAMP(1);
+  LYRA_HSTAMP(0, 1);
 
   const int wn = wave & 3, wm = wave >> 2;
 
@@ -137,6 +139,7 @@
   }
   LYRA_WG_END();
   LYRA_TSTAMP(6);
+  LYRA_HSTAMP(0, 2);
   LYRA_WSTAMP(101);
   l2_warm_sink(warm, state, B);
   l2_warm_sink(warm_code, state, B);
@@ -155,9 +158,11 @@
   const int m = lane & 15, q = lane >> 4;
   const int b0 = tile * S1;
   LYRA_TSTAMP(70);
+  LYRA_HSTAMP(1, 0);
   LYRA_WSTAMP(102);
   int my_id = 0;
   if (tid < S1) my_id = ids[min(b0 + tid, B - 1)];
+  const int id_me = slot_id(ids, b0, (tid >> 5) & (S1 - 1), B);
   constexpr int XIN = (4 * S1 * 32) / NT1;
   static_assert((4 * S1 * 32) % NT1 == 0 && (4 * S1 * 32) / NT1 >= 1, "the unrolled input prefetch covers the stage input only when the thread count divides it");
   f32x4 xin[XIN];
@@ -172,29 +177,39 @@
     sids[tid] = my_id;
     sphase[tid] = *reinterpret_cast<const int*>(state + (size_t)max(my_id, 0) * st::E1_BYTES + st::PHASE);
   }
-  const auto warm = l2_warm<NT1, 2>(P.warm);
-  const auto warm_code = code_warm<NT1>(code_bytes);
-#pragma unroll
-  for (int k = 0; k < XIN; ++k) {
-    const int idx = tid + k * NT1;
-    int p4 = idx & 31, s = (idx >> 5) & (S1 - 1), t = (idx >> 5) / S1;
-    *reinterpret_cast<f32x4*>(&XB[((2 + t) * S1 + s) * CS1 + p4 * 4]) = xin[k];
-  }
-  LYRA_SYNC_KEEP();
   auto soff = [&](int s) -> uint32_t { return (uint32_t)max(sids[s], 0) * (uint32_t)st::E1_BYTES; };
   auto gat = [&](uint32_t o) -> uint8_t LYRA_GLOBAL* { return (uint8_t LYRA_GLOBAL*)state + o; };
   auto valid = [&](int s) -> bool { return b0 + s < B && sids[s] >= 0; };
-
   TileCtx cx{state, sids, sphase, B - b0, st::E1_BYTES};
-  const auto H0 = hist128_prefetch<S1, NT1>(cx, 1, st::E_R1_0);
-  for (int idx = tid; idx < 2 * S1 * 32; idx += NT1) {
+  const uint32_t so_me = slot_off(id_me, st::E1_BYTES);
+  const auto H0 = hist128_prefetch_at<S1, NT1>(cx, so_me, 0, 1, st::E_R1_0);
+  constexpr int DIN = (2 * S1 * 32) / NT1;
+  static_assert((2 * S1 * 32) % NT1 == 0 && DIN >= 1 && (NT1 >> 5) % S1 == 0, "one slot per thread");
+  f32x4 din[DIN];
+#pragma unroll
+  for (int k = 0; k < DIN; ++k) {
+    const int idx = tid + k * NT1;
+    int p4 = idx & 31, j = (idx >> 5) / S1;
+    din[k] = *(const f32x4 LYRA_GLOBAL*)gat(so_me + (uint32_t)(st::E_D1 + (j * 128 + p4 * 4) * 4));
+  }
+  const auto warm = l2_warm<NT1, 2>(P.warm);
+  const auto warm_code = code_warm<NT1>(code_bytes);
+#pragma unroll
+  for (int k = 0; k < XIN; ++k) {
+    const int idx = tid + k * NT1;
+    int p4 = idx & 31, s = (idx >> 5) & (S1 - 1), t = (idx >> 5) / S1;
+    *reinterpret_cast<f32x4*>(&XB[((2 + t) * S1 + s) * CS1 + p4 * 4]) = xin[k];
+  }
+#pragma unroll
+  for (int k = 0; k < DIN; ++k) {
+    const int idx = tid + k * NT1;
     int p4 = idx & 31, s = (idx >> 5) & (S1 - 1), j = (idx >> 5) / S1;
-    *reinterpret_cast<f32x4*>(&XB[(j * S1 + s) * CS1 + p4 * 4]) =
-        *(const f32x4 LYRA_GLOBAL*)gat(soff(s) + (uint32_t)(st::E_D1 + (j * 128 + p4 * 4) * 4));
-  }
-  __syncthreads();
+    *reinterpret_cast<f32x4*>(&XB[(j * S1 + s) * CS1 + p4 * 4]) = din[k];
+  }
+  LYRA_SYNC_KEEP();
 
   LYRA_TSTAMP(71);
+  LYRA_HSTAMP(1, 1);
   resblocks128<S1, NT1>(XB + 2 * S1 * CS1, DB, PB, cx, P.dw, P.pw, P.cv, st::E_R1_0, st::E_R1_1, st::E_R1_2, H0);
 
   LYRA_TSTAMP(72);
@@ -243,6 +258,7 @@
     }
   }
   LYRA_TSTAMP(73);
+  LYRA_HSTAMP(1, 2);
   LYRA_WSTAMP(103);
   if (tid < S1 && valid(tid)) {
     int ph = sphase[tid] + 1;
diff --git a/lyra_amd/csrc/kernels.h b/lyra_amd/csrc/kernels.h
--- a/lyra_amd/csrc/kernels.h
+++ b/lyra_amd/csrc/kernels.h
@@ -21,8 +21,11 @@
 #ifndef LYRA_PFB_DEC_S2
 #define LYRA_PFB_DEC_S2 4
 #endif
+#ifndef LYRA_PFB_ENC_S2
+#define LYRA_PFB_ENC_S2 2
+#endif
 constexpr int PFB_ENC_S0 = LYRA_PFB_ENC_S0, PFB_ENC_S1 = LYRA_PFB_ENC_S1, PFB_DEC_S1 = LYRA_PFB_DEC_S1,
-              PFB_DEC_S2 = LYRA_PFB_DEC_S2;
+              PFB_DEC_S2 = LYRA_PFB_DEC_S2, PFB_ENC_S2 = LYRA_PFB_ENC_S2;
 
 struct EncS0P { ConvF first; DwF dw[3]; ConvF pw[3]; ConvF cv[3]; ConvF down; WarmRange warm; };
 struct EncS1P { DwF dw[3]; ConvF pw[3]; ConvF cv[3]; ConvF down; WarmRange warm; };
diff --git a/lyra_amd/csrc/lyra_dev.h b/lyra_amd/csrc/lyra_dev.h
--- a/lyra_amd/csrc/lyra_dev.h
+++ b/lyra_amd/csrc/lyra_dev.h
@@ -23,7 +23,12 @@
     g_lyra_wgtrace[blockIdx.x * 4 + 2] = __builtin_amdgcn_s_getreg(63492); \
     g_lyra_wgtrace[blockIdx.x * 4 + 3] = __builtin_amdgcn_s_getreg(63508); } } while (0)
 #define LYRA_WG_END() do { if (threadIdx.x == 0 && blockIdx.x < 2048) g_lyra_wgtrace[blockIdx.x * 4 + 1] = wall_clock64(); } while (0)
+static __device__ long long g_lyra_heads[3 * 128 * 4];
+#define LYRA_HSTAMP(slot, k) do { if (threadIdx.x == 0 && blockIdx.x % 17 == 0 && blockIdx.x / 17 < 128) { \
+    long long* h_ = &g_lyra_heads[((slot) * 128 + blockIdx.x / 17) * 4]; h_[k] = clock64(); \
+    if ((k) == 0) h_[3] = __builtin_amdgcn_s_getreg(63508); } } while (0)
 #else
+#define LYRA_HSTAMP(slot, k) do { } while (0)
 #define LYRA_WG_BEGIN() do { } while (0)
 #define LYRA_WG_END() do { } while (0)
 #define LYRA_WSTAMP(i) do { } while (0)
diff --git a/lyra_amd/csrc/resblocks.h b/lyra_amd/csrc/resblocks.h
--- a/lyra_amd/csrc/resblocks.h
+++ b/lyra_amd/csrc/resblocks.h
@@ -18,6 +18,9 @@
   }
 };
 
+__device__ __forceinline__ int slot_id(const int32_t* ids, int b0, int s, int B) { return as_global(ids)[min(b0 + s, B - 1)]; }
+__device__ __forceinline__ uint32_t slot_off(int id, int stride) { return (uint32_t)max(id, 0) * (uint32_t)stride; }
+
 template <int S, int NT>
 __device__ __forceinline__ uint32_t state_touch(const TileCtx& cx, int off, int bytes) {
   const int l0 = off >> 7, n = ((off + bytes - 1) >> 7) - l0 + 1;
@@ -26,6 +29,17 @@
   if (idx < S * n) {
     const int s = idx / n, l = idx - s * n;
     tok = *cx.at<const uint32_t>(cx.soff(s) + (uint32_t)((l0 + l) << 7));
+  }
+  return tok;
+}
+template <int S, int NT>
+__device__ __forceinline__ uint32_t state_touch_head(uint8_t* state, const int32_t* ids, int b0, int B, int stride, int off, int bytes) {
+  const int l0 = off >> 7, n = ((off + bytes - 1) >> 7) - l0 + 1;
+  const int idx = threadIdx.x;
+  uint32_t tok = 0;
+  if (idx < S * n) {
+    const int s = idx / n, l = idx - s * n;
+    tok = *(const uint32_t LYRA_GLOBAL*)((uint8_t LYRA_GLOBAL*)state + (slot_off(slot_id(ids, b0, s, B), stride) + (uint32_t)((l0 + l) << 7)));
   }
   return tok;
 }
@@ -143,13 +157,13 @@
 struct Hist128 { f32x4 h[RPT][2]; };
 
 template <int S, int NT>
-__device__ __forceinline__ Hist128<1024 / NT> hist128_prefetch(const TileCtx& cx, int d, int off) {
+__device__ __forceinline__ Hist128<1024 / NT> hist128_prefetch_at(const TileCtx& cx, uint32_t soff, int phase, int d, int off) {
   constexpr int RPT = 1024 / NT;
-  const int tid = threadIdx.x, p4 = tid & 31, s = (tid >> 5) & (S - 1), row0 = (tid >> 8) * RPT;
+  const int tid = threadIdx.x, p4 = tid & 31, row0 = (tid >> 8) * RPT;
   const int R2 = 2 * d;
   const bool ring = R2 > 4;
-  const int base = ring ? (cx.sphase[s] * 4) % R2 : 0;
-  const uint32_t hp = cx.soff(s) + (uint32_t)(off + p4 * 16);
+  const int base = ring ? (phase * 4) % R2 : 0;
+  const uint32_t hp = soff + (uint32_t)(off + p4 * 16);
   Hist128<RPT> H;
 #pragma unroll
   for (int k = 0; k < RPT; ++k)
@@ -164,6 +178,11 @@
       }
     }
   return H;
+}
+template <int S, int NT>
+__device__ __forceinline__ Hist128<1024 / NT> hist128_prefetch(const TileCtx& cx, int d, int off) {
+  const int s = (threadIdx.x >> 5) & (S - 1);
+  return hist128_prefetch_at<S, NT>(cx, cx.soff(s), 2 * d > 4 ? cx.sphase[s] : 0, d, off);
 }
 
 template <int S, int NT>
```

After: 14.41 million. No clear change (-0.3%).
